# DefaultRui/VLN-VER

Measured on AMD Instinct MI355X. Metric: viewpoints/sec (multi-view->voxel fwd+bwd), vocc.py config, higher is better.
Workload: dtype bf16

## Files before the change

### include/ver_ops.h

```cpp
#ifndef VER_OPS_H
#define VER_OPS_H

#include <stdint.h>

#ifdef __cplusplus
extern "C" {
#endif

#define VER_ABI_VERSION 31

#define VER_OK            0
#define VER_EINVAL       -1
#define VER_EUNSUPPORTED -2
#define VER_ELAUNCH      -3

#define VER_F32  0
#define VER_BF16 1

int         ver_abi_version(void);
const char* ver_last_error(void);

int ver_msda_forward(const float* value, const int64_t* shapes_hw, const int64_t* level_start,
                     const float* loc, const float* attn_w, float* out,
                     int B, int num_keys, int heads, int head_dim, int levels, int points,
                     int Nq, int im2col_step, void* stream);

int ver_msda_backward(const float* value, const int64_t* shapes_hw, const int64_t* level_start,
                      const float* loc, const float* attn_w, const float* grad_out,
                      float* grad_value, float* grad_loc, float* grad_attn_w,
                      int B, int num_keys, int heads, int head_dim, int levels, int points,
                      int Nq, int im2col_step, void* stream);

int ver_msda3d_forward(const float* value, const int64_t* shapes_dhw, const int64_t* level_start,
                       const float* loc, const float* attn_w, float* out,
                       int B, int num_keys, int heads, int head_dim, int levels, int points,
                       int Nq, void* stream);
int ver_msda3d_backward(const float* value, const int64_t* shapes_dhw, const int64_t* level_start,
                        const float* loc, const float* attn_w, const float* grad_out,
                        float* grad_value, float* grad_loc, float* grad_attn_w,
                        int B, int num_keys, int heads, int head_dim, int levels, int points,
                        int Nq, void* stream);


int ver_project_points(const float* world2pixel, const float* origin, const float* pc_range,
                       int B, int Ncam, int bev_z, int bev_h, int bev_w,
                       float img_w, float img_h,
                       float* uv, uint8_t* vis, int32_t* vis_list, int32_t* vis_cnt,
                       int32_t* zero_list, int32_t* zero_cnt, int32_t* fwd_list, int32_t* fwd_cnt,
                       void* stream);

int ver_hits_from_mask(const uint8_t* bev_mask, int B, int Ncam, int Nq, int D,
                       uint8_t* vis, int32_t* vis_list, int32_t* vis_cnt,
                       int32_t* zero_list, int32_t* zero_cnt, int32_t* fwd_list, int32_t* fwd_cnt,
                       void* stream);

#define VER_SCA_ROWS_PREZEROED 1
#define VER_SCA_VALUE_HEAD_MAJOR 2
#define VER_SCA_GRAD_SLOTS_BF16 4
int ver_sca_head_major_supported(int value_dtype, int head_dim, int points, int map_h, int map_w);
int ver_sca_zero_rows(const int32_t* zero_list, const int32_t* zero_cnt, float* slots, int B, int Nq, int row_floats,
                      void* stream);
int ver_sca_forward(const void* value, int value_dtype, const float* offsets, const float* logits,
                    const float* uv, const uint8_t* vis, const int32_t* vis_list,
                    const int32_t* vis_cnt, const int32_t* zero_list, const int32_t* zero_cnt,
                    const int32_t* fwd_list, const int32_t* fwd_cnt,
                    float* slots,
                    int B, int Ncam, int Nq, int D, int heads, int head_dim, int points,
                    int map_h, int map_w, int flags, void* stream);

int ver_sca_backward_grad_dtype(int value_dtype, int head_dim, int points, int map_h, int map_w);
int ver_sca_backward(const void* value, int value_dtype, const float* offsets, const float* logits,
                     const float* uv, const uint8_t* vis, const int32_t* vis_list,
                     const int32_t* vis_cnt, const int32_t* fwd_list, const int32_t* fwd_cnt,
                     const void* grad_slots,
                     void* grad_value, int grad_value_dtype, float* grad_offsets, float* grad_logits,
                     int B, int Ncam, int Nq, int D, int heads, int head_dim, int points,
                     int map_h, int map_w, int flags, void* stream);

int ver_lattice_im2col(const void* src, void* col, const int* taps, int ntaps,
                       int B, int Z, int H, int W, int C, int dtype, void* stream);
int ver_lattice_col2im(const void* grad_col, void* grad_src, const int* taps, int ntaps,
                       int B, int Z, int H, int W, int C, int dtype, void* stream);

int ver_lattice_gather(const void* src, void* col, const int* taps, const long* col_offset, long col_stride,
                       int ntaps, int B, int Zr, int Zs, int H, int W, int C, int layout, int dtype,
                       const void* const_rows, const long* const_offset, int const_blocks, int const_width, void* stream);
int ver_lattice_scatter(const void* grad_col, void* grad_src, const int* taps, const long* col_offset,
                        long col_stride, int ntaps, int B, int Zr, int Zs, int H, int W, int C, int layout, int dtype,
                        void* stream);

int ver_convt_weight_forward(const float* weight, void* taps, long pairs, int dtype, void* stream);
int ver_convt_weight_backward(const void* grad_taps, float* grad_weight, long pairs, int dtype, void* stream);
int ver_convt_weight_backward_blocks(const void* blocks, const long* block_offsets, long ld, const void* prev_bias,
                                     const void* grad_v, float* grad_weight, int ci, int co, int dtype, void* stream);
int ver_convt_weight_forward_blocks(const float* weight, const long* block_offsets, long ld, void* blocks, int ci, int co,
                                    int dtype, void* stream);
int ver_blocks_vec_forward(const void* blocks, const long* block_rows, int nblocks, long ld, int ci, int ncols, const float* x,
                           float* vec, int dtype, void* stream);
int ver_blocks_vec_backward(const void* blocks, const long* block_rows, int nblocks, long ld, int ci, int ncols,
                            const float* grad_vec, float* grad_x, int dtype, void* stream);
int ver_lattice_transpose(void* channels_last, void* channel_first, long cf_stride, int B, int Z, int H, int W,
                          int C, int layout, int to_channel_first, int dtype, void* stream);
int ver_lattice_rows(void* channels_last, void* rows, long quarter, int period, int nseg, const int* seg_off,
                     const int* seg_len, const long* seg_base, const int* seg_pitch, const int* seg_rows, int B, int Z,
                     int H, int W, int C, int layout, int to_rows, int dtype, void* stream);

int ver_ln_relu_forward(const void* x, const float* gamma, const float* beta, void* y,
                        float* mean, float* rstd, long N, int W, float eps, int dtype, void* stream);
int ver_ln_relu_backward(const void* x, const void* grad_y, const float* gamma, const float* beta,
                         const float* mean, const float* rstd, void* grad_x,
                         float* grad_gamma, float* grad_beta, long N, int W, int dtype, void* stream);

int ver_focal_loss_blocks(long N, int C);
int ver_focal_loss_forward(const void* logits, const int64_t* target, float* partial, long N, int C,
                           float gamma, float alpha, int dtype, int32_t* bad_labels, void* stream);
int ver_focal_loss_forward_grad(const void* logits, const int64_t* target, float* partial, void* grad, long N, int C,
                                float gamma, float alpha, int dtype, int32_t* bad_labels, void* stream);
int ver_focal_loss_forward_grad_u8(const void* logits, const uint8_t* target, float* partial, void* grad, long N, int C,
                                   float gamma, float alpha, int dtype, int32_t* bad_labels, void* stream);
int ver_focal_loss_backward(const void* logits, const int64_t* target, const float* scale, void* grad,
                            long N, int C, float gamma, float alpha, int dtype, void* stream);

int ver_add_ln_forward(const void* a, int a_dtype, const float* residual, const float* gamma, const float* beta,
                       const int64_t* seed, float p_drop, float eps, float* y, void* y_bf16, float* mean,
                       float* rstd, long N, int C, void* stream);
int ver_add_ln_backward(const float* grad_y, const void* grad_y_bf16, const void* a, int a_dtype,
                        const float* residual, const float* gamma, const float* mean, const float* rstd,
                        const int64_t* seed, float p_drop, void* grad_a, float* grad_residual, float* grad_gamma,
                        float* grad_beta, long N, int C, void* stream);
int ver_relu_dropout_forward(const void* x, void* y, const int64_t* seed, float p_drop, long n, int dtype, void* stream);
int ver_relu_dropout_backward(const void* y, const void* grad_y, void* grad_x, float p_drop, long n, int dtype,
                              void* stream);

int ver_run_gather(const void* image, long image_stride, const int32_t* run_start, const int32_t* aug_idx,
                   void* rows, int B, int n_rows, int runs, int run_len, int n_aug, int row_elems, int dtype,
                   void* stream);
int ver_run_scatter(const void* rows, void* image, long image_stride, const int32_t* run_start, int B,
                    int n_rows, int runs, int run_len, int row_elems, int dtype, void* stream);

#define VER_OCC_MLP_CENTERED 2
long ver_occ_mlp_image_bytes(void);
int ver_occ_mlp_vector_floats(void);
int ver_occ_mlp_pack(const float* W1, const float* W2, const float* W3, void* image, void* stream);
int ver_occ_mlp_forward(const void* x, const void* image, const float* vectors, void* logits,
                        long N, int width, int classes, float eps, int first_linear, void* stream);
int ver_occ_mlp_forward_stats(const void* x, const void* image, const float* vectors, void* logits, float* rstd,
                              long N, int width, int classes, float eps, int first_linear, void* stream);
int ver_occ_mlp_backward(const void* x, const void* grad_logits, const void* image, const float* vectors,
                         void* grad_x, void* grad_a1, void* grad_a2, void* h1,
                         float* param_grads, long N, int width, int classes, float eps, int first_linear,
                         void* stream);
int ver_occ_mlp_backward_fused(const void* x, const void* grad_logits, const float* W2, const float* W3,
                               const float* vectors, void* grad_x, float* param_grads, long N, int width,
                               int classes, float eps, const float* grad_scale, int flags, void* stream);
int ver_occ_mlp_backward_fused_stats(const void* x, const void* grad_logits, const float* W2, const float* W3,
                                     const float* vectors, const float* rstd, void* grad_x, float* param_grads, long N,
                                     int width, int classes, float eps, const float* grad_scale, int flags, void* stream);

long ver_occ_predict_blocks(long N);
int  ver_occ_predict(const void* logits, int dtype, long N, int C, float threshold, int32_t* block_work,
                     int64_t* pairs, int64_t* count, void* stream);

int  ver_occ_confusion(const void* logits, int dtype, long rows_per_sample, int samples, int C, const uint8_t* labels,
                       const float* thresholds, int num_thresholds, int64_t* hist, void* stream);

int  ver_wgrad_tn_splits(long M, int Ka, int N);
int  ver_wgrad_tn_splits_ld(long M, int Ka, int N, long ld);
long ver_wgrad_tn_workspace(long M, int Ka, int N, int splits);
int  ver_wgrad_tn(const void* a, long lda, const void* g, long ldg, long M, int Ka, int N, void* out, long ldo,
                  int out_dtype, int splits, int flags, void* workspace, long workspace_bytes, void* stream);
int  ver_wgrad_tn_segments(const void* lattice, int layout, int B, int H, int W, int C, const int* taps, int nseg, const void* cst,
                           int ncst, int cw, const void* g, long ldg, int N, void* out, long ldo, int out_dtype, int splits,
                           void* workspace, long workspace_bytes, void* stream);
int  ver_wgrad_tn_segments_splits(int B, int H, int W, long Ka, int N, long ldg);

int  ver_gemm_nn(const void* a, long lda, const void* w, long ldw, const float* bias, void* c, long ldc, long M, int K,
                 int N, int flags, void* stream);
int  ver_gemm_nn_taps(const void* lattice, int layout, int B, int H, int W, int C, const int* taps, int ntaps, const void* w,
                      long ldw, const float* rowpos, const float* bias, void* c, long ldc, int N, void* stream);
int  ver_gemm_nn_segments(const void* lattice, int layout, int B, int H, int W, int C, const int* taps, int ntaps,
                          const void* cst, int ncst, int cw, const void* w, long ldw, const float* rowpos, const float* bias,
                          void* c, long ldc, int N, void* stream);
int  ver_gemm_nn_planes(const void* lattice, int layout, int B, int H, int W, int C, long plane_elems, int nplanes,
                        const int* tap_plane, const int* taps, int ntaps, const void* cst, int ncst, int cw, const void* w,
                        long ldw, const float* rowpos, const float* bias, void* c, long ldc, int N, void* stream);
int  ver_gemm_nn_splits(long M, int K, int N);
int  ver_gemm_nn_splitk(const void* a, long lda, const void* w, long ldw, const float* bias, void* c, long ldc, long M, int K,
                        int N, int splits, void* workspace, long workspace_bytes, void* stream);

int ver_clip_adamw_step(void* const* table, const long* sizes, const int* chunk_tensor, const int* chunk_index,
                        int n_tensors, int n_chunks, int chunk_elems, float* partial, float* norm_out, float max_norm,
                        float lr, float beta1, float beta2, float eps, float weight_decay, long step, void* stream);

int ver_clip_adamw_step_tensors(void* const* table, const long* sizes, const int* chunk_tensor, const int* chunk_index,
                                const float* hyper, int* steps, int n_tensors, int n_chunks, int chunk_elems, float* partial,
                                float* norm_out, float max_norm, void* stream);

int ver_lsa_solve(const float* cost, const int32_t* ncols, int32_t* match, int32_t* bad,
                  int P, int R, int Ccap, void* stream);

#ifdef __cplusplus
}
#endif
#endif
```

### vln-ver_amd/csrc/ver_wgrad.hip

```cpp
#include <cstdlib>
#include "ver_common.h"

namespace {
typedef __bf16 bf16x8 __attribute__((ext_vector_type(8)));
typedef float f32x16 __attribute__((ext_vector_type(16)));
typedef short s16x4 __attribute__((ext_vector_type(4)));
typedef short s16x8 __attribute__((ext_vector_type(8)));
typedef __attribute__((address_space(3))) s16x4 lds_s16x4;
typedef __attribute__((address_space(3))) void lds_void;

constexpr int kTile = 256;
constexpr int kSlabRows = 16;
constexpr int kSlabBytes = 2 * kSlabRows * kTile * 2;
constexpr int kRing = 8;
constexpr int kLdsBytes = kRing * kSlabBytes;

typedef int i32x2 __attribute__((ext_vector_type(2)));
typedef int i32x4 __attribute__((ext_vector_type(4)));

template <int OFF>
__device__ __forceinline__ i32x2 tr_read(int addr) {
    i32x2 v;
    asm volatile("ds_read_b64_tr_b16 %0, %1 offset:%2" : "=v"(v) : "v"(addr), "n"(OFF) : "memory");
    return v;
}
__device__ __forceinline__ bf16x8 frag(i32x2 lo, i32x2 hi) {
    return __builtin_bit_cast(bf16x8, (i32x4)__builtin_shufflevector(lo, hi, 0, 1, 2, 3));
}

struct WgradArgs {
    const __bf16* A;
    const __bf16* G;
    float* ws;
    long lda, ldg, M, Mc;
    int S, Ka, N, tiles_n, T;
    void* out;
    long ldo;
    int out_bf16;
    const __bf16* lattice;
    long lattice_bytes;
    const __bf16* cst;
    long cst_bytes;
    int B, H, W, C, P, CW, ncst, nseg;
    int seg_start[65];
    signed char kind[64], dz[64], dy[64], dx[64];
};

constexpr int kOutsideW = (int)0x80000000;
template <int L>
__device__ __forceinline__ int wcell_off(const WgradArgs& t, int b, int zl, int y, int x, int dz) {
    if ((unsigned)y >= (unsigned)t.H || (unsigned)x >= (unsigned)t.W) return kOutsideW;
    const int j = dz >> 1;
    int v;
    if (L == 0)
        v = ((b * 4 + zl + dz) * t.H + y) * t.W + x;
    else if (L == 2)
        v = ((((b * 2 + zl) * t.H + y) * t.W + x) << 1) + j;
    else
        v = (((((((y & 1) << 1 | (x & 1)) * t.B + b) * 2 + zl) * (t.H >> 1) + (y >> 1)) * (t.W >> 1) + (x >> 1)) << 1) + j;
    return v * t.C * 2;
}

struct WTapLane {
    int taddr;
    int boff;
    int bstep;
    int pend;
    int tend;
    int rows_left;
    int vo;
};

template <int L>
__device__ __forceinline__ int wtap_table_entry(const WgradArgs& t, int seg, int pos) {
    if (seg < 0) return kOutsideW;
    if (t.kind[seg]) return (pos * t.ncst + t.dz[seg]) * t.CW * 2;
    const int hw = t.H * t.W;
    const int zl = pos / hw, rem = pos - zl * hw;
    const int y = rem / t.W, x = rem - y * t.W;
    return wcell_off<L>(t, 0, zl, y + t.dy[seg], x + t.dx[seg], t.dz[seg]);
}

__device__ __forceinline__ int lds_read_b32(int addr) {
    int v;
    asm volatile("ds_read_b32 %0, %1" : "=v"(v) : "v"(addr) : "memory");
    return v;
}

__device__ __forceinline__ void wtap_step(const WgradArgs& t, WTapLane& tl, int tfetched) {
    tl.boff += tl.pend;
    tl.rows_left -= kSlabRows;
    tl.vo = tl.rows_left > 0 ? (int)((unsigned)tfetched + (unsigned)tl.boff) : kOutsideW;
    tl.taddr += 4 * kSlabRows;
    tl.pend = 0;
    if (tl.taddr >= tl.tend) tl.taddr -= 4 * t.P, tl.pend = tl.bstep;
}

struct WgradLane {
    int offA0, offA1, offB0, offB1;
    int voA, voG;
    int stepA, stepG;
    int dmaoff;
};

template <int SLOT>
__device__ __forceinline__ void read_slab(const WgradLane& c, i32x2 (&al)[4], i32x2 (&ah)[4], i32x2 (&bl)[2], i32x2 (&bh)[2]) {
    constexpr int SB = (SLOT & 3) * kSlabBytes;
    constexpr int UP = SLOT >= 4 ? 65536 : 0;
    const int a0 = c.offA0 + UP, a1 = c.offA1 + UP, b0 = c.offB0 + UP, b1 = c.offB1 + UP;
    al[0] = tr_read<SB>(a0);
    ah[0] = tr_read<SB + 512>(a0);
    bl[0] = tr_read<SB>(b0);
    bh[0] = tr_read<SB + 512>(b0);
    al[1] = tr_read<SB>(a1);
    ah[1] = tr_read<SB + 512>(a1);
    bl[1] = tr_read<SB>(b1);
    bh[1] = tr_read<SB + 512>(b1);
    al[2] = tr_read<SB + 1024>(a0);
    ah[2] = tr_read<SB + 1536>(a0);
    al[3] = tr_read<SB + 1024>(a1);
    ah[3] = tr_read<SB + 1536>(a1);
}

template <int PS, int KP, int PF, int IMPL>
__device__ __forceinline__ void phase(char* lds, f32x16 (&acc)[4][2], const WgradLane& c, __amdgpu_buffer_rsrc_t ra,
                                      __amdgpu_buffer_rsrc_t rg, unsigned& soA, unsigned& soG, const WgradArgs& t, WTapLane& tl) {
    i32x2 al[KP][4], ah[KP][4], bl[KP][2], bh[KP][2];
    int tnext = 0;
    read_slab<PS * KP>(c, al[0], ah[0], bl[0], bh[0]);
    if constexpr (KP == 2) read_slab<PS * KP + 1>(c, al[KP - 1], ah[KP - 1], bl[KP - 1], bh[KP - 1]);
#pragma unroll
    for (int u = 0; u < KP; ++u) {
        const int ds = (PS * KP + u + PF) % kRing;
        if constexpr (IMPL < 0) {
            __builtin_amdgcn_raw_ptr_buffer_load_lds(ra, (lds_void*)(lds + ds * kSlabBytes + c.dmaoff), 16, c.voA, (int)soA, 0, 0);
        } else {
            static_assert(IMPL < 0 || KP == 1, "implicit A: one slab per phase");
            __builtin_amdgcn_raw_ptr_buffer_load_lds(ra, (lds_void*)(lds + ds * kSlabBytes + c.dmaoff), 16, tl.vo, 0, 0, 0);
            tnext = lds_read_b32(tl.taddr);
        }
        __builtin_amdgcn_raw_ptr_buffer_load_lds(rg, (lds_void*)(lds + ds * kSlabBytes + kSlabBytes / 2 + c.dmaoff), 16, c.voG, (int)soG, 0, 0);
        soA += (unsigned)c.stepA;
        soG += (unsigned)c.stepG;
    }
    asm volatile("s_waitcnt vmcnt(%0)" ::"n"(2 * (PF - KP)) : "memory");
    __builtin_amdgcn_s_barrier();
    asm volatile("s_waitcnt lgkmcnt(0)"
                 : "+v"(al[0][0]), "+v"(ah[0][0]), "+v"(al[0][1]), "+v"(ah[0][1]), "+v"(al[0][2]), "+v"(ah[0][2]), "+v"(al[0][3]),
                   "+v"(ah[0][3]), "+v"(bl[0][0]), "+v"(bh[0][0]), "+v"(bl[0][1]), "+v"(bh[0][1]), "+v"(tnext)
                 :
                 : "memory");

    if constexpr (KP == 2)
        asm volatile(""
                     : "+v"(al[KP - 1][0]), "+v"(ah[KP - 1][0]), "+v"(al[KP - 1][1]), "+v"(ah[KP - 1][1]), "+v"(al[KP - 1][2]),
                       "+v"(ah[KP - 1][2]), "+v"(al[KP - 1][3]), "+v"(ah[KP - 1][3]), "+v"(bl[KP - 1][0]), "+v"(bh[KP - 1][0]),
                       "+v"(bl[KP - 1][1]), "+v"(bh[KP - 1][1])
                     :
                     : "memory");
    bf16x8 a[KP][4], b[KP][2];
#pragma unroll
    for (int u = 0; u < KP; ++u) {
#pragma unroll
        for (int i = 0; i < 4; ++i) a[u][i] = frag(al[u][i], ah[u][i]);
        b[u][0] = frag(bl[u][0], bh[u][0]);
        b[u][1] = frag(bl[u][1], bh[u][1]);
    }
    __builtin_amdgcn_sched_barrier(0);
    __builtin_amdgcn_s_setprio(1);
#pragma unroll
    for (int u = 0; u < KP; ++u)
#pragma unroll
        for (int it = 0; it < 4; ++it)
#pragma unroll
            for (int jt = 0; jt < 2; ++jt)
                acc[it][jt] = __builtin_amdgcn_mfma_f32_32x32x16_bf16(a[u][it], b[u][jt], acc[it][jt], 0, 0, 0);
    __builtin_amdgcn_s_setprio(0);
    __builtin_amdgcn_sched_barrier(0);
    if constexpr (IMPL >= 0) {
        wtap_step(t, tl, tnext);
        __builtin_amdgcn_sched_barrier(0);
    }
    __builtin_amdgcn_s_barrier();
}

template <int PS, int KP, int PF, int IMPL>
__device__ __forceinline__ void phases_from(int left, char* lds, f32x16 (&acc)[4][2], const WgradLane& c,
                                            __amdgpu_buffer_rsrc_t ra, __amdgpu_buffer_rsrc_t rg, unsigned& soA, unsigned& soG,
                                            const WgradArgs& t, WTapLane& tl) {
    if constexpr (PS < kRing / KP) {
        if (left > PS * KP) {
            phase<PS, KP, PF, IMPL>(lds, acc, c, ra, rg, soA, soG, t, tl);
            phases_from<PS + 1, KP, PF, IMPL>(left, lds, acc, c, ra, rg, soA, soG, t, tl);
        }
    }
}

template <int KP, int PF, int IMPL>
__device__ __forceinline__ void wgrad_body(const WgradArgs& p) {
    static_assert(PF >= KP && PF + (KP == 1 ? 2 : 4) <= kRing, "prefetch distance against the ring (WAR on the slot)");
    extern __shared__ __attribute__((aligned(1024))) char lds[];
    const int tid = threadIdx.x, lane = tid & 63;
    const int wave = __builtin_amdgcn_readfirstlane(tid >> 6);
    const int wr = wave >> 2, wc = wave & 3;
    int chunk, tile;
    {
        const int b = blockIdx.x;
        if ((p.S & 7) == 0) {
            const int xcd = b & 7, idx = b >> 3;
            chunk = xcd + 8 * (idx / p.T);
            tile = idx % p.T;
        } else {
            chunk = b / p.T;
            tile = b % p.T;
        }
    }
    const int mt = tile / p.tiles_n, nt = tile - mt * p.tiles_n;
    const long row0 = (long)chunk * p.Mc;
    const long rows = max(0L, min(p.Mc, p.M - row0));
    const int nslab = (int)((rows + kSlabRows * KP - 1) / (kSlabRows * KP)) * KP;

    const __bf16* ab = IMPL < 0 ? p.A + row0 * p.lda + (long)mt * kTile : nullptr;
    const __bf16* gb = p.G + row0 * p.ldg + (long)nt * kTile;
    const long abytes = ((p.M - row0 - 1) * p.lda + p.Ka - (long)mt * kTile) * 2;
    const long gbytes = ((p.M - row0 - 1) * p.ldg + p.N - (long)nt * kTile) * 2;
    const __amdgpu_buffer_rsrc_t rg = __builtin_amdgcn_make_buffer_rsrc((void*)gb, 0, (int)max(0L, min(gbytes, 0xFFFFFFFFL)), 0x00020000);
    WgradLane c;
    const int prow = lane >> 3, pch = (lane & 7) ^ (((prow >> 1) & 1) << 2);
    WTapLane tl = {};
    bool a_cst = false;
    if constexpr (IMPL >= 0) {
        int* tables = reinterpret_cast<int*>(lds + kLdsBytes);
        auto seg_of = [&](int col0) {
            int seg = -1;
            for (int i = 0; i < p.nseg; ++i)
                if (col0 >= p.seg_start[i] && col0 < p.seg_start[i + 1]) seg = i;
            return seg;
        };
        for (int q = 0; q < 4; ++q) {
            const int seg = seg_of(mt * kTile + 64 * q);
            for (int i = tid; i < p.P; i += 512) tables[q * p.P + i] = wtap_table_entry<IMPL>(p, seg, i);
        }
        __syncthreads();
        const int col0 = mt * kTile + 64 * (wave & 3);
        const int seg = seg_of(col0);
        a_cst = seg >= 0 && p.kind[seg];
        const long r = row0 + 8 * (wave >> 2) + prow;
        const int b0 = (int)(r / p.P), pos0 = (int)(r - (long)b0 * p.P);
        tl.bstep = a_cst ? 0 : (IMPL == 3 ? p.H * p.W : 4 * p.H * p.W) * p.C * 2;
        tl.boff = b0 * tl.bstep + (seg < 0 ? 0 : (col0 - p.seg_start[seg]) * 2) + pch * 16;
        const int lbase = (int)(uintptr_t)(__attribute__((address_space(3))) char*)(lds + kLdsBytes) + (wave & 3) * p.P * 4;
        tl.tend = lbase + 4 * p.P;
        tl.taddr = lbase + 4 * pos0;
        tl.pend = 0;
        tl.rows_left = (int)min(min(p.M, row0 + p.Mc) - r, 0x7FFFFFF0L) + kSlabRows;
        int t0 = lds_read_b32(tl.taddr);
        asm volatile("s_waitcnt lgkmcnt(0)" : "+v"(t0)::"memory");
        wtap_step(p, tl, t0);
    }
    const __amdgpu_buffer_rsrc_t ra =
        IMPL < 0 ? __builtin_amdgcn_make_buffer_rsrc((void*)ab, 0, (int)max(0L, min(abytes, 0xFFFFFFFFL)), 0x00020000)
                 : __builtin_amdgcn_make_buffer_rsrc((void*)(a_cst ? p.cst : p.lattice), 0,
                                                     (int)max(0L, min(a_cst ? p.cst_bytes : p.lattice_bytes, 0x7FFFFFFFL)), 0x00020000);
    c.voA = (int)(((8 * (wave >> 2) + prow) * p.lda + 64 * (wave & 3)) * 2) + pch * 16;
    c.voG = (int)(((8 * (wave >> 2) + prow) * p.ldg + 64 * (wave & 3)) * 2) + pch * 16;
    c.stepA = (int)(kSlabRows * p.lda * 2);
    c.stepG = (int)(kSlabRows * p.ldg * 2);
    c.dmaoff = wave * 1024;
    unsigned soA = 0, soG = 0;

    {
        const int q = lane >> 4, cl = lane & 15;
        const int lowch = (2 * (q & 1) + ((cl & 3) >> 1)) ^ (((cl >> 3) & 1) << 2);
        const int lbase = (int)(uintptr_t)(__attribute__((address_space(3))) char*)lds;
        const int rowoff = lbase + ((q >> 1) * 32 + (cl >> 2)) * 128 + lowch * 16 + (cl & 1) * 8;
        c.offA0 = rowoff + 2 * wr * 1024;
        c.offA1 = c.offA0 ^ 64;
        c.offB0 = rowoff + wc * 1024 + kSlabBytes / 2;
        c.offB1 = c.offB0 ^ 64;
    }

    f32x16 acc[4][2];
#pragma unroll
    for (int it = 0; it < 4; ++it)
#pragma unroll
        for (int jt = 0; jt < 2; ++jt)
#pragma unroll
            for (int r = 0; r < 16; ++r) acc[it][jt][r] = 0.0f;

#pragma unroll
    for (int s = 0; s < PF; ++s) {
        if constexpr (IMPL < 0) {
            __builtin_amdgcn_raw_ptr_buffer_load_lds(ra, (lds_void*)(lds + s * kSlabBytes + c.dmaoff), 16, c.voA, (int)soA, 0, 0);
        } else {
            __builtin_amdgcn_raw_ptr_buffer_load_lds(ra, (lds_void*)(lds + s * kSlabBytes + c.dmaoff), 16, tl.vo, 0, 0, 0);
            int tn = lds_read_b32(tl.taddr);
            asm volatile("s_waitcnt lgkmcnt(0)" : "+v"(tn)::"memory");
            wtap_step(p, tl, tn);
        }
        __builtin_amdgcn_raw_ptr_buffer_load_lds(rg, (lds_void*)(lds + s * kSlabBytes + kSlabBytes / 2 + c.dmaoff), 16, c.voG, (int)soG, 0, 0);
        soA += (unsigned)c.stepA;
        soG += (unsigned)c.stepG;
    }
    asm volatile("s_waitcnt vmcnt(%0)" ::"n"(2 * (PF - KP)) : "memory");
    __builtin_amdgcn_s_barrier();
    if (wr == 1) __builtin_amdgcn_s_barrier();

    int s = 0;
    for (; s + kRing <= nslab; s += kRing) phases_from<0, KP, PF, IMPL>(kRing, lds, acc, c, ra, rg, soA, soG, p, tl);
    phases_from<0, KP, PF, IMPL>(nslab - s, lds, acc, c, ra, rg, soA, soG, p, tl);
    if (wr == 0) __builtin_amdgcn_s_barrier();
    asm volatile("s_waitcnt vmcnt(0)" ::: "memory");

    const int i0 = mt * kTile + 128 * wr + 4 * (lane >> 5), j0 = nt * kTile + 64 * wc + (lane & 31);
    if (p.S == 1 && p.out) {
#pragma unroll
        for (int it = 0; it < 4; ++it)
#pragma unroll
            for (int jt = 0; jt < 2; ++jt) {
                const int j = j0 + 32 * jt;
#pragma unroll
                for (int r = 0; r < 16; ++r) {
                    const int i = i0 + 32 * it + (r & 3) + 8 * (r >> 2);
                    if (i < p.Ka && j < p.N) {
                        if (p.out_bf16)
                            reinterpret_cast<__bf16*>(p.out)[(long)i * p.ldo + j] = (__bf16)acc[it][jt][r];
                        else
                            reinterpret_cast<float*>(p.out)[(long)i * p.ldo + j] = acc[it][jt][r];
                    }
                }
            }
        return;
    }
    float* out = p.ws + (long)chunk * p.Ka * p.N;
#pragma unroll
    for (int it = 0; it < 4; ++it)
#pragma unroll
        for (int jt = 0; jt < 2; ++jt) {
            const int j = j0 + 32 * jt;
#pragma unroll
            for (int r = 0; r < 16; ++r) {
                const int i = i0 + 32 * it + (r & 3) + 8 * (r >> 2);
                if (i < p.Ka && j < p.N) out[(long)i * p.N + j] = acc[it][jt][r];
            }
        }
}

template <int KP, int PF>
__global__ __launch_bounds__(512) void k_wgrad_tn(WgradArgs p) {
    wgrad_body<KP, PF, -1>(p);
}

template <int L, int PF>
__global__ __launch_bounds__(512) void k_wgrad_tn_seg(WgradArgs p) {
    wgrad_body<1, PF, L>(p);
}

template <typename OT>
__global__ __launch_bounds__(256) void k_wgrad_reduce(const float* __restrict__ ws, OT* __restrict__ out, long ldo, int S,
                                                      int Ka, int N) {
    const long n4 = (long)Ka * N / 4;
    const long stride = (long)Ka * N;
    for (long e = blockIdx.x * 256L + threadIdx.x; e < n4; e += (long)gridDim.x * 256) {
        float4 acc = *reinterpret_cast<const float4*>(ws + 4 * e);
        for (int s = 1; s < S; ++s) {
            const float4 v = *reinterpret_cast<const float4*>(ws + s * stride + 4 * e);
            acc.x += v.x;
            acc.y += v.y;
            acc.z += v.z;
            acc.w += v.w;
        }
        const long i = (4 * e) / N, j = (4 * e) - i * N;
        OT* o = out + i * ldo + j;
        if constexpr (sizeof(OT) == 4) {
            *reinterpret_cast<float4*>(o) = acc;
        } else {
            typedef __bf16 bf16x4 __attribute__((ext_vector_type(4)));
            bf16x4 v;
            v.x = (__bf16)acc.x;
            v.y = (__bf16)acc.y;
            v.z = (__bf16)acc.z;
            v.w = (__bf16)acc.w;
            *reinterpret_cast<bf16x4*>(o) = v;
        }
    }
}

long max_chunk_rows(long ld) {
    if (ld <= 0) return 45000;
    const long rows = (0xFFFFFFFFL / (ld * 2)) - 16 * kRing - 2 * kSlabRows - 1;
    return rows < 45000 ? (rows > 2 * kSlabRows ? rows : 2 * kSlabRows) : 45000;
}

int pick_splits(long M, int Ka, int N, long ld = 0) {
    const long cap = max_chunk_rows(ld);
    const long tiles = (long)((Ka + kTile - 1) / kTile) * ((N + kTile - 1) / kTile);
    static const int cand[] = {1, 2, 3, 4, 6, 8, 12, 16, 24, 32, 48, 64};
    int best = 0;
    double best_us = 0.0;
    for (int s : cand) {
        if ((M + s - 1) / s > cap) continue;
        if (s > 1 && M / s < 256) break;
        if (M > 32768 && s % 8) continue;
        const long rounds = (tiles * s + 255) / 256;
        const double slabs = (double)((M + s - 1) / s + 15) / 16.0;
        double us = (double)rounds * (slabs * 0.37 + 8.0) + (s == 1 ? 0.25 : (double)s) * (double)Ka * (double)N * 8.0 / 3.0e6;
        if (s % 8 == 0) us *= 0.97;
        if (!best || us < best_us) {
            best = s;
            best_us = us;
        }
    }
    if (!best) {
        best = 64;
        while (best < 65536 && (M + best - 1) / best > cap) best *= 2;
    }
    return best;
}

template <int KP, int PF>
void launch_tn(const WgradArgs& p, int blocks, hipStream_t st, hipError_t& e) {
    auto kern = k_wgrad_tn<KP, PF>;
    e = hipFuncSetAttribute((const void*)kern, hipFuncAttributeMaxDynamicSharedMemorySize, kLdsBytes);
    if (e == hipSuccess) hipLaunchKernelGGL(kern, dim3((unsigned)blocks), dim3(512), kLdsBytes, st, p);
}
template <int L, int PF>
void launch_tn_segments_pf(const WgradArgs& p, int blocks, hipStream_t st, hipError_t& e) {
    const int ldsb = kLdsBytes + 4 * p.P * 4;
    e = hipFuncSetAttribute((const void*)k_wgrad_tn_seg<L, PF>, hipFuncAttributeMaxDynamicSharedMemorySize, ldsb);
    if (e == hipSuccess) hipLaunchKernelGGL((k_wgrad_tn_seg<L, PF>), dim3((unsigned)blocks), dim3(512), ldsb, st, p);
}

template <int L>
void launch_tn_segments(const WgradArgs& p, int blocks, hipStream_t st, hipError_t& e) {
    static const int pf = [] {
        const char* v = getenv("VER_WGRAD_SEG_PF");
        return v ? atoi(v) : 3;
    }();
    if (pf == 4) launch_tn_segments_pf<L, 4>(p, blocks, st, e);
    else if (pf == 5) launch_tn_segments_pf<L, 5>(p, blocks, st, e);
    else if (pf == 6) launch_tn_segments_pf<L, 6>(p, blocks, st, e);
    else launch_tn_segments_pf<L, 3>(p, blocks, st, e);
}
}

extern "C" int ver_wgrad_tn_splits(long M, int Ka, int N) {
    if (M <= 0 || Ka <= 0 || N <= 0) return 1;
    return pick_splits(M, Ka, N);
}

extern "C" int ver_wgrad_tn_splits_ld(long M, int Ka, int N, long ld) {
    if (M <= 0 || Ka <= 0 || N <= 0) return 1;
    return pick_splits(M, Ka, N, ld);
}

extern "C" long ver_wgrad_tn_workspace(long M, int Ka, int N, int splits) {
    if (Ka <= 0 || N <= 0) return 0;
    if (splits <= 0) splits = ver_wgrad_tn_splits(M, Ka, N);
    return (long)splits * Ka * N * (long)sizeof(float);
}

extern "C" int ver_wgrad_tn(const void* a, long lda, const void* g, long ldg, long M, int Ka, int N, void* out, long ldo,
                            int out_dtype, int splits, int flags, void* workspace, long workspace_bytes, void* stream) {
    hipStream_t st = (hipStream_t)stream;
    VER_REQUIRE(M >= 0 && Ka > 0 && N > 0, VER_EINVAL, "ver_wgrad_tn: bad sizes M=%ld Ka=%d N=%d", M, Ka, N);
    VER_REQUIRE(out && workspace && ((a && g) || M == 0), VER_EINVAL, "ver_wgrad_tn: null pointer argument");
    VER_REQUIRE(out_dtype == VER_F32 || out_dtype == VER_BF16, VER_EINVAL, "ver_wgrad_tn: out_dtype %d", out_dtype);
    VER_REQUIRE(lda >= Ka && ldg >= N && ldo >= N, VER_EINVAL, "ver_wgrad_tn: row pitch smaller than the row");
    VER_REQUIRE(lda % 8 == 0 && ldg % 8 == 0 && ((uintptr_t)a & 15) == 0 && ((uintptr_t)g & 15) == 0, VER_EUNSUPPORTED,
                "ver_wgrad_tn: operands must be 16-byte aligned with row pitches that are multiples of 8 elements");
    VER_REQUIRE(N % 4 == 0 && ldo % 4 == 0 && ((uintptr_t)out & 15) == 0, VER_EUNSUPPORTED,
                "ver_wgrad_tn: N and the output pitch must be multiples of 4");
    const int S = splits > 0 ? splits : pick_splits(M, Ka, N, lda > ldg ? lda : ldg);
    VER_REQUIRE(S <= 65536, VER_EINVAL, "ver_wgrad_tn: %d row chunks", S);
    const long Mc = ((M + S - 1) / S + 2 * kSlabRows - 1) / (2 * kSlabRows) * (2 * kSlabRows);
    VER_REQUIRE((Mc + 16 * kRing) * (lda > ldg ? lda : ldg) * 2 < 0xFFFFFFFFL, VER_EUNSUPPORTED,
                "ver_wgrad_tn: a row chunk exceeds the 4-GiB range of a buffer offset (more splits)");
    VER_REQUIRE(workspace_bytes >= (long)S * Ka * N * (long)sizeof(float), VER_EINVAL, "ver_wgrad_tn: workspace of %ld bytes, %ld needed",
                workspace_bytes, (long)S * Ka * N * (long)sizeof(float));
    WgradArgs p = {};
    p.A = (const __bf16*)a;
    p.G = (const __bf16*)g;
    p.ws = (float*)workspace;
    p.lda = lda;
    p.ldg = ldg;
    p.M = M;
    p.Mc = Mc;
    p.S = S;
    p.Ka = Ka;
    p.N = N;
    p.tiles_n = (N + kTile - 1) / kTile;
    p.T = ((Ka + kTile - 1) / kTile) * p.tiles_n;
    const bool direct = S == 1 && M > 0;
    p.out = direct ? out : nullptr;
    p.ldo = ldo;
    p.out_bf16 = out_dtype == VER_BF16;
    hipError_t e = hipSuccess;
    if (M > 0) {
        switch (flags & 15) {
            case 4: launch_tn<1, 4>(p, p.T * S, st, e); break;
            case 5: launch_tn<1, 5>(p, p.T * S, st, e); break;
            case 6: launch_tn<1, 6>(p, p.T * S, st, e); break;
            case 8 + 2: launch_tn<2, 2>(p, p.T * S, st, e); break;
            case 8 + 4: launch_tn<2, 4>(p, p.T * S, st, e); break;
            default: launch_tn<1, 3>(p, p.T * S, st, e); break;
        }
        if (e != hipSuccess) return ver_fail(VER_ELAUNCH, "ver_wgrad_tn: LDS attribute: %s", hipGetErrorString(e));
    } else if (int zrc = ver_zero_async(workspace, (size_t)S * Ka * N * sizeof(float), st)) {
        return zrc;
    }
    if (direct) return ver_check_launch("ver_wgrad_tn");
    const long n4 = (long)Ka * N / 4;
    long grid = (n4 + 255) / 256;
    if (grid > 8192) grid = 8192;
    if (out_dtype == VER_F32)
        hipLaunchKernelGGL(k_wgrad_reduce<float>, dim3((unsigned)grid), dim3(256), 0, st, (const float*)workspace, (float*)out, ldo, S, Ka, N);
    else
        hipLaunchKernelGGL(k_wgrad_reduce<__bf16>, dim3((unsigned)grid), dim3(256), 0, st, (const float*)workspace, (__bf16*)out, ldo, S, Ka, N);
    return ver_check_launch("ver_wgrad_tn");
}

extern "C" int ver_wgrad_tn_segments(const void* lattice, int layout, int B, int H, int W, int C, const int* taps, int nseg,
                                     const void* cst, int ncst, int cw, const void* g, long ldg, int N, void* out, long ldo,
                                     int out_dtype, int splits, void* workspace, long workspace_bytes, void* stream) {
    hipStream_t st = (hipStream_t)stream;
    VER_REQUIRE(B >= 0 && H > 0 && W > 0 && C > 0 && N > 0 && nseg > 0, VER_EINVAL, "ver_wgrad_tn_segments: bad sizes");
    VER_REQUIRE(layout == 0 || layout == 2 || layout == 3, VER_EINVAL, "ver_wgrad_tn_segments: layout %d (0 plain, 2 z-split, 3 planar z-split)", layout);
    VER_REQUIRE(layout != 3 || (H % 2 == 0 && W % 2 == 0), VER_EINVAL, "ver_wgrad_tn_segments: planar needs even H, W");
    VER_REQUIRE(out && workspace && ((lattice && g && taps) || B == 0), VER_EINVAL, "ver_wgrad_tn_segments: null pointer argument");
    VER_REQUIRE(out_dtype == VER_F32 || out_dtype == VER_BF16, VER_EINVAL, "ver_wgrad_tn_segments: out_dtype %d", out_dtype);
    VER_REQUIRE(nseg <= 64, VER_EUNSUPPORTED, "ver_wgrad_tn_segments: %d segments (at most 64)", nseg);
    VER_REQUIRE(C % 64 == 0 && (cst == nullptr || (ncst > 0 && ncst <= 64 && cw > 0 && cw % 64 == 0 && ((uintptr_t)cst & 15) == 0)),
                VER_EUNSUPPORTED, "ver_wgrad_tn_segments: segment widths (C = %d, pattern blocks of %d) must be multiples of 64", C, cw);
    const long M = (long)B * 2 * H * W, lbytes = (long)B * 4 * H * W * C * 2;
    const int P = 2 * H * W;
    VER_REQUIRE(P >= kSlabRows && P <= 2048 && lbytes < 0x7FFFFFFFL, VER_EUNSUPPORTED,
                "ver_wgrad_tn_segments: %d rows per viewpoint / a source lattice of %ld bytes (16 <= rows <= 2048: four offset tables "
                "next to the 128-KB ring in LDS; below 2 GiB)", P, lbytes);
    VER_REQUIRE(ldg >= N && ldo >= N && ldg % 8 == 0 && ((uintptr_t)g & 15) == 0 && ((uintptr_t)lattice & 15) == 0, VER_EUNSUPPORTED,
                "ver_wgrad_tn_segments: g must be 16-byte aligned with a row pitch that is a multiple of 8 elements");
    VER_REQUIRE(N % 4 == 0 && ldo % 4 == 0 && ((uintptr_t)out & 15) == 0, VER_EUNSUPPORTED,
                "ver_wgrad_tn_segments: N and the output pitch must be multiples of 4");
    WgradArgs p = {};
    long Ka = 0;
    for (int i = 0; i < nseg; ++i) {
        const int dz = taps[3 * i], dy = taps[3 * i + 1], dx = taps[3 * i + 2];
        p.seg_start[i] = (int)Ka;
        if (dz < 0) {
            VER_REQUIRE(cst && -1 - dz < ncst, VER_EINVAL, "ver_wgrad_tn_segments: segment %d names pattern block %d of %d", i, -1 - dz, cst ? ncst : 0);
            p.kind[i] = 1, p.dz[i] = (signed char)(-1 - dz);
            Ka += cw;
        } else {
            VER_REQUIRE((dz == 0 || dz == 2) && dy >= -64 && dy <= 64 && dx >= -64 && dx <= 64, VER_EINVAL,
                        "ver_wgrad_tn_segments: tap %d = (%d, %d, %d): dz must be 0 or 2", i, dz, dy, dx);
            p.kind[i] = 0, p.dz[i] = (signed char)dz, p.dy[i] = (signed char)dy, p.dx[i] = (signed char)dx;
            Ka += C;
        }
    }
    p.seg_start[nseg] = (int)Ka;
    VER_REQUIRE(Ka < 0x7FFFFFFFL, VER_EUNSUPPORTED, "ver_wgrad_tn_segments: %ld columns", Ka);
    const int S = splits > 0 ? splits : pick_splits(M, (int)Ka, N, ldg);
    VER_REQUIRE(S <= 65536, VER_EINVAL, "ver_wgrad_tn_segments: %d row chunks", S);
    const long Mc = ((M + S - 1) / S + 2 * kSlabRows - 1) / (2 * kSlabRows) * (2 * kSlabRows);
    VER_REQUIRE((Mc + 16 * kRing) * ldg * 2 < 0xFFFFFFFFL, VER_EUNSUPPORTED,
                "ver_wgrad_tn_segments: a row chunk exceeds the 4-GiB range of a buffer offset (more splits)");
    VER_REQUIRE(workspace_bytes >= (long)S * Ka * N * (long)sizeof(float), VER_EINVAL, "ver_wgrad_tn_segments: workspace of %ld bytes, %ld needed",
                workspace_bytes, (long)S * Ka * N * (long)sizeof(float));
    p.A = nullptr;
    p.G = (const __bf16*)g;
    p.ws = (float*)workspace;
    p.lda = 0;
    p.ldg = ldg;
    p.M = M;
    p.Mc = Mc;
    p.S = S;
    p.Ka = (int)Ka;
    p.N = N;
    p.tiles_n = (N + kTile - 1) / kTile;
    p.T = (int)((Ka + kTile - 1) / kTile) * p.tiles_n;
    const bool direct = S == 1 && M > 0;
    p.out = direct ? out : nullptr;
    p.ldo = ldo;
    p.out_bf16 = out_dtype == VER_BF16;
    p.lattice = (const __bf16*)lattice;
    p.lattice_bytes = lbytes;
    p.cst = (const __bf16*)cst;
    p.cst_bytes = cst ? (long)P * ncst * cw * 2 : 0;
    p.B = B, p.H = H, p.W = W, p.C = C, p.P = P, p.CW = cw, p.ncst = ncst, p.nseg = nseg;
    hipError_t e = hipSuccess;
    if (M > 0) {
        if (layout == 0) launch_tn_segments<0>(p, p.T * S, st, e);
        else if (layout == 2) launch_tn_segments<2>(p, p.T * S, st, e);
        else launch_tn_segments<3>(p, p.T * S, st, e);
        if (e != hipSuccess) return ver_fail(VER_ELAUNCH, "ver_wgrad_tn_segments: LDS attribute: %s", hipGetErrorString(e));
    } else if (int zrc = ver_zero_async(workspace, (size_t)S * Ka * N * sizeof(float), st)) {
        return zrc;
    }
    if (direct) return ver_check_launch("ver_wgrad_tn_segments");
    const long n4 = Ka * N / 4;
    long grid = (n4 + 255) / 256;
    if (grid > 8192) grid = 8192;
    if (out_dtype == VER_F32)
        hipLaunchKernelGGL(k_wgrad_reduce<float>, dim3((unsigned)grid), dim3(256), 0, st, (const float*)workspace, (float*)out, ldo, S, (int)Ka, N);
    else
        hipLaunchKernelGGL(k_wgrad_reduce<__bf16>, dim3((unsigned)grid), dim3(256), 0, st, (const float*)workspace, (__bf16*)out, ldo, S, (int)Ka, N);
    return ver_check_launch("ver_wgrad_tn_segments");
}

extern "C" int ver_wgrad_tn_segments_splits(int B, int H, int W, long Ka, int N, long ldg) {
    const long M = (long)B * 2 * H * W;
    if (M <= 0 || Ka <= 0 || N <= 0) return 1;
    return pick_splits(M, (int)Ka, N, ldg);
}
```

### vln-ver_amd/dense_heads/upsample.py

```python
import os

import torch

from . import _cpu_algebra
from ._cpu_algebra import ZS_PLAIN, ZS_PLANAR_SPLIT, ZS_SPLIT, planar_to_plain, planar_zs_to_plain, zs_to_plain
from ._cpu_algebra import plain_to_planar
from .lattice_plan import (_CLASSES, _COLS3, _COLS4, _PW, _PW2, _aug_rows_z4, _block_offsets, _class_patterns, _class_rows_z4,
                           _class_segments_z4, _const_rows_z4, _dgrad_plan, _layer0_z4_plan, _layer_plan, _layer_plan_z4,
                           _stack_tables_z4)

KERNEL = (3, 5, 5)
GEOM = dict(stride=(1, 2, 2), padding=(2, 4, 4), dilation=(2, 2, 2), output_padding=(0, 1, 1))
_HIP_DTYPES = (torch.float32, torch.bfloat16)


class _HipAlgebra:

    @staticmethod
    def corr_weight(weight, dtype):
        if weight.dtype == torch.float32 and dtype in _HIP_DTYPES:
            from ..hipops import convt_weight_taps
            return convt_weight_taps(weight, dtype)
        return _cpu_algebra.corr_weight(weight, dtype)

    @staticmethod
    def im2col(e, taps):
        from ..hipops import lattice_im2col
        return lattice_im2col(e.contiguous(), taps)

    @staticmethod
    def gather27(e, planar, a_mat, ci, hc, wc, taps, offs):
        from ..hipops import lattice_gather
        lattice_gather(e.contiguous(), a_mat, taps, offs, (hc, wc), 1 if planar else 0)

    @staticmethod
    def scatter27(d_a, planar, shape, ci, hc, wc, taps, offs):
        from ..hipops import lattice_scatter
        return lattice_scatter(d_a, d_a.new_empty(shape), taps, offs, (hc, wc), 1 if planar else 0)

    @staticmethod
    def gather_z4(e, layout, a_mat, taps, offs, ci, hc, wc, const=None):
        from ..hipops import lattice_gather
        if const is not None and e.dtype in _HIP_DTYPES:
            lattice_gather(e.contiguous(), a_mat, taps, offs, (hc, wc), layout, row_z=2, const_rows=const[0], const_offset=const[1])
            return True
        lattice_gather(e.contiguous(), a_mat, taps, offs, (hc, wc), layout, row_z=2)
        return False

    @staticmethod
    def scatter_z4(d_a, layout, shape, taps, offs, ci, hc, wc):
        from ..hipops import lattice_scatter
        return lattice_scatter(d_a, d_a.new_empty(shape), taps, offs, (hc, wc), layout, row_z=2)

    @staticmethod
    def channels_last(x0, dt):
        b, c, z, h, w = x0.shape
        pos = z * h * w
        if dt in _HIP_DTYPES:
            vx = 4 if dt == torch.bfloat16 else 2
            for wd in range(min(pos, 120), 0, -1):
                if pos % wd == 0 and wd % vx == 0:
                    return _ChannelsLast.apply(x0, dt, (pos // wd, wd))
        return _cpu_algebra.channels_last(x0, dt)


def _algebra(t):
    return _HipAlgebra if t.is_cuda else _cpu_algebra


def _on_hip(t):
    return _algebra(t) is _HipAlgebra


def is_reference_geometry(conv):
    return (tuple(conv.kernel_size) == KERNEL and tuple(conv.stride) == GEOM['stride'] and
            tuple(conv.padding) == GEOM['padding'] and tuple(conv.dilation) == GEOM['dilation'] and
            tuple(conv.output_padding) == GEOM['output_padding'] and conv.groups == 1)


_to_plain, _from_plain = _cpu_algebra.to_plain, _cpu_algebra.from_plain


def _corr_weight(weight, dtype):
    return _algebra(weight).corr_weight(weight, dtype)


def _im2col(e, taps):
    return _algebra(e).im2col(e, taps)


def _bias_through_taps(prev_bias, k):
    t, ci, _ = k.shape
    return torch.bmm(prev_bias.view(1, 1, ci).expand(t, 1, ci).contiguous(), k).squeeze(1)


def _stacked_rows(k, bias, prev_bias, total_rows):
    _, ci, co = k.shape
    v = _bias_through_taps(prev_bias.to(k.dtype), k)
    vaug = torch.cat([v, bias.to(k.dtype)[None], v.new_zeros(_PW - 76, co)])
    return torch.cat([k.reshape(75 * ci, co), vaug, vaug, vaug, vaug, v.new_zeros(total_rows - 75 * ci - 4 * _PW, co)])


def _stacked_rows_backward(d_rows, k, prev_bias):
    _, ci, co = k.shape
    dt = k.dtype
    n_data = 75 * ci
    acc = torch.float64 if dt == torch.float64 else torch.float32
    d_vaug = d_rows[n_data:n_data + 4 * _PW].view(4, _PW, co).sum(0, dtype=acc)
    d_v = d_vaug[:75].to(dt)
    d_k = torch.addcmul(d_rows[:n_data].view(75, ci, co), prev_bias.to(dt)[None, :, None], d_v[:, None, :])
    d_prev = torch.bmm(k, d_v.unsqueeze(2)).sum(0).squeeze(1)
    return d_k, d_vaug[75].to(prev_bias.dtype), d_prev.to(prev_bias.dtype)


def _layer0(e, k, bias):
    b, z, h, w, c = e.shape
    taps = [(2 * a - 2, bb - 2, cc - 2) for a in range(3) for bb in range(5) for cc in range(5)]
    a_mat = _im2col(e, taps)
    out = torch.addmm(bias, a_mat, k.reshape(75 * c, -1))
    return out.view(b, z, h, w, -1)


def _gather27(e, planar, a_mat, ci, hc, wc):
    _algebra(e).gather27(e, planar, a_mat, ci, hc, wc, _COLS3.taps, _COLS3.block_offsets(ci))


def _scatter27(d_a, planar, shape, ci, hc, wc):
    return _algebra(d_a).scatter27(d_a, planar, shape, ci, hc, wc, _COLS3.taps, _COLS3.block_offsets(ci))


class _LatticeLayer(torch.autograd.Function):

    @staticmethod
    def forward(ctx, e, k, bias, prev_bias, planar):
        if planar:
            _, b, z, hh, wh, ci = e.shape
            hc, wc = 2 * hh, 2 * wh
        else:
            b, z, hc, wc, ci = e.shape
        co = k.shape[-1]
        plan, kt, total_rows = _layer_plan(ci, e.device)
        m = b * z * hc * wc
        a_mat = e.new_empty(m, kt)
        _gather27(e, planar, a_mat, ci, hc, wc)
        a3 = a_mat.view(b, z * hc * wc, kt)
        for cls, pat in zip(_CLASSES, _class_patterns(z, hc, wc, e.device, e.dtype)):
            o = _COLS3.const_offset(cls, ci)
            a3[:, :, o:o + _PW] = pat
        rows = _stacked_rows(k, bias, prev_bias, total_rows)
        out = e.new_empty(4, m, co)
        for p, cls in enumerate(_CLASSES):
            c0, c1, ridx = plan[cls]
            torch.mm(a_mat[:, c0:c1], rows.index_select(0, ridx), out=out[p])
        ctx.save_for_backward(a_mat, rows, k, prev_bias)
        ctx.geom = (planar, tuple(e.shape), hc, wc)
        return out.view(4, b, z, hc, wc, co)

    @staticmethod
    def backward(ctx, grad_out):
        a_mat, rows, k, prev_bias = ctx.saved_tensors
        planar, e_shape, hc, wc = ctx.geom
        _, ci, co = k.shape
        plan, kt, total_rows = _layer_plan(ci, a_mat.device)
        m = a_mat.shape[0]
        g = grad_out.contiguous().view(4, m, co)
        d_a = a_mat.new_empty(m, kt)
        d_a[:, kt - _PW:] = 0
        d_rows = rows.new_empty(total_rows, co)
        for p, cls in enumerate(_CLASSES):
            c0, c1, ridx = plan[cls]
            w = rows.index_select(0, ridx)
            if p == 0:
                torch.mm(g[p], w.t(), out=d_a[:, c0:c1])
            else:
                torch.addmm(d_a[:, c0:c1], g[p], w.t(), out=d_a[:, c0:c1])
            d_rows.index_copy_(0, ridx, rows_tn(a_mat[:, c0:c1], g[p]))
        d_e = _scatter27(d_a, planar, e_shape, ci, hc, wc)
        return (d_e, *_stacked_rows_backward(d_rows, k, prev_bias), None)


def _gather_z4(e, layout, a_mat, taps, offs, ci, hc, wc, with_const=False):
    const = _const_rows_z4(ci, hc, wc, e.device, e.dtype) if with_const else None
    return _algebra(e).gather_z4(e, layout, a_mat, taps, offs, ci, hc, wc, const)


def _scatter_z4(d_a, layout, shape, taps, offs, ci, hc, wc):
    return _algebra(d_a).scatter_z4(d_a, layout, shape, taps, offs, ci, hc, wc)


_IMPLICIT_TAPS = os.environ.get('VER_IMPLICIT_TAPS', '1') != '0'


def _implicit_taps(e, layout, rows, combined_hw, ci, raw, const_width):
    if not (_IMPLICIT_TAPS and _OWN_GEMM and raw is not None and _on_hip(e) and e.dtype == torch.bfloat16 and rows >= _OWN_GEMM_MIN_ROWS):
        return False
    from ..hipops import gemm_nn_taps_supported, wgrad_tn_segments_supported
    return gemm_nn_taps_supported(e, layout, None, ci) and wgrad_tn_segments_supported(e, layout, combined_hw, ci, const_width, None)


def _dgrad_implicit(kind, g_planes, weights, b, hc, wc, ci, co):
    from ..hipops import gemm_nn_taps
    lat = g_planes.view(g_planes.shape[0], b, 2, hc, wc, 2, co)
    rows, taps, planes, nb = _dgrad_plan(kind, ci, g_planes.device)
    wcat = weights.index_select(0, rows).view(nb, 2 * ci, 2 * co).transpose(1, 2).reshape(nb * 2 * co, 2 * ci)
    d_e = gemm_nn_taps(lat if kind != 'l0' else lat[0], ZS_SPLIT, (hc, wc), taps, wcat, planes=planes if kind != 'l0' else None,
                       timer_class='head_gemm_dgrad')
    return d_e.view(b, 2, hc, wc, 2, ci)


def _dgrad_explicit_l0(g, wmat, shape, taps, offs, ci, h, w):
    with gemm_timed('head_gemm_dgrad', g.shape[0], g.shape[1], wmat.shape[0]):
        d_a = torch.mm(g, wmat.t())
    return _scatter_z4(d_a, ZS_PLAIN, shape, taps, offs, ci, h, w)


class _Layer0Z4Taps(torch.autograd.Function):

    @staticmethod
    def forward(ctx, x, k, bias):
        b, _, h, w, ci = x.shape
        co = k.shape[-1]
        taps, offs, lo, hi = _layer0_z4_plan(ci, x.device)
        a_mat = x.new_empty(b * 2 * h * w, 50 * ci)
        _gather_z4(x, ZS_PLAIN, a_mat, taps, offs, ci, h, w)
        rows = k.reshape(75 * ci, co)
        wmat = torch.cat([rows.index_select(0, lo), rows.index_select(0, hi)], 1)
        out = mm_fwd(a_mat, wmat, bias=torch.cat([bias, bias]))
        ctx.save_for_backward(a_mat, wmat)
        ctx.geom = (tuple(x.shape), ci, co, h, w)
        return out.view(b, 2, h, w, 2, co)

    @staticmethod
    def backward(ctx, grad_out):
        a_mat, wmat = ctx.saved_tensors
        shape, ci, co, h, w = ctx.geom
        taps, offs, lo, hi = _layer0_z4_plan(ci, a_mat.device)
        g = grad_out.contiguous().view(-1, 2 * co)
        d_x = _dgrad_explicit_l0(g, wmat, shape, taps, offs, ci, h, w)
        d_w = rows_tn(a_mat, g)
        d_b = g.sum(0, dtype=torch.float64 if g.dtype == torch.float64 else torch.float32)
        d_lo = d_w.new_zeros(75 * ci, co)
        d_hi = d_w.new_zeros(75 * ci, co)
        d_lo.index_copy_(0, lo, d_w[:, :co])
        d_hi.index_copy_(0, hi, d_w[:, co:])
        return d_x, (d_lo + d_hi).view(75, ci, co), (d_b[:co] + d_b[co:]).to(g.dtype)


class _Layer0Z4Raw(torch.autograd.Function):

    @staticmethod
    def forward(ctx, x, raw, bias):
        from ..hipops import convt_weight_forward_blocks
        b, _, h, w, ci = x.shape
        co = raw.shape[1]
        taps, offs, _, _ = _layer0_z4_plan(ci, x.device)
        ctx.implicit = _implicit_taps(x, ZS_PLAIN, b * 2 * h * w, (h, w), ci, raw, 0)
        if ctx.implicit:
            operand = x.contiguous()
        else:
            operand = x.new_empty(b * 2 * h * w, 50 * ci)
            _gather_z4(x, ZS_PLAIN, operand, taps, offs, ci, h, w)
        wmat = convt_weight_forward_blocks(raw, _block_offsets('l0', ci, co, x.device), x.new_empty(50 * ci, 2 * co), ci, co)
        bias2 = torch.cat([bias, bias])
        if ctx.implicit:
            from ..hipops import gemm_nn_taps
            out = gemm_nn_taps(operand, ZS_PLAIN, (h, w), taps, wmat, bias=bias2.to(x.dtype).float())
        else:
            out = mm_fwd(operand, wmat, bias=bias2)
        ctx.save_for_backward(operand, wmat)
        ctx.geom = (tuple(x.shape), ci, co, h, w)
        return out.view(b, 2, h, w, 2, co)

    @staticmethod
    def backward(ctx, grad_out):
        from ..hipops import convt_weight_backward_blocks
        operand, wmat = ctx.saved_tensors
        shape, ci, co, h, w = ctx.geom
        taps, offs, _, _ = _layer0_z4_plan(ci, operand.device)
        g = grad_out.contiguous().view(-1, 2 * co)
        if ctx.implicit:
            from ..hipops import wgrad_tn_segments
            d_x = zs_to_plain(_dgrad_implicit('l0', g[None], wmat, shape[0], h, w, ci, co))
            d_w = wgrad_tn_segments(operand, ZS_PLAIN, (h, w), taps, g)
        else:
            d_x = _dgrad_explicit_l0(g, wmat, shape, taps, offs, ci, h, w)
            d_w = rows_tn(operand, g)
        d_b = g.sum(0, dtype=torch.float32)
        d_raw = convt_weight_backward_blocks(d_w, _block_offsets('l0', ci, co, d_w.device), None, None, ci, co)
        return d_x, d_raw, (d_b[:co] + d_b[co:]).to(g.dtype)


def _geom_z4(e, planar):
    if planar:
        _, b, _, hh, wh, _, ci = e.shape
        return ZS_PLANAR_SPLIT, b, 2 * hh, 2 * wh, ci
    b, _, hc, wc, _, ci = e.shape
    return ZS_SPLIT, b, hc, wc, ci


def _tap_matrix_z4(e, layout, b, hc, wc, ci):
    _, kt, _, taps, offs = _layer_plan_z4(ci, e.device)
    a_mat = e.new_empty(b * 2 * hc * wc, kt)
    if not _gather_z4(e, layout, a_mat, taps, offs, ci, hc, wc, with_const=True):
        a3 = a_mat.view(b, 2 * hc * wc, kt)
        for cls, pat in zip(_CLASSES, _class_patterns(4, hc, wc, e.device, e.dtype)):
            o = _COLS4.const_offset(cls, ci)
            halves = pat.view(2, 2 * hc * wc, _PW)
            a3[:, :, o:o + _PW] = halves[0]
            a3[:, :, o + _PW:o + _PW2] = halves[1]
    return a_mat


def _class_ranges_z4(ci, device):
    plan, rows = _layer_plan_z4(ci, device)[0], _class_rows_z4(ci)
    ranges = [(plan[cls][0], plan[cls][1], rows[cls][0], rows[cls][0] + plan[cls][1] - plan[cls][0]) for cls in _CLASSES]
    return ranges, ranges[-1][3]


def _dgrad_class(d_a, p, g_p, w, c0, c1):
    with gemm_timed('head_gemm_dgrad', g_p.shape[0], g_p.shape[1], c1 - c0):
        if p == 0:
            torch.mm(g_p, w.t(), out=d_a[:, c0:c1])
        else:
            torch.addmm(d_a[:, c0:c1], g_p, w.t(), out=d_a[:, c0:c1])


class _LatticeLayerZ4Taps(torch.autograd.Function):

    @staticmethod
    def forward(ctx, e, k, bias, prev_bias, planar):
        layout, b, hc, wc, ci = _geom_z4(e, planar)
        co = k.shape[-1]
        plan, _, total_rows, _, _ = _layer_plan_z4(ci, e.device)
        a_mat = _tap_matrix_z4(e, layout, b, hc, wc, ci)
        out = e.new_empty(4, a_mat.shape[0], 2 * co)
        rows = _stacked_rows(k, bias, prev_bias, total_rows)
        ws = []
        for p, cls in enumerate(_CLASSES):
            c0, c1, _, _, lohi = plan[cls]
            ws.append(rows.index_select(0, lohi).view(c1 - c0, 2 * co))
            mm_fwd(a_mat[:, c0:c1], ws[p], out=out[p])
        ctx.save_for_backward(a_mat, k, prev_bias, *ws)
        ctx.geom = (layout, tuple(e.shape), hc, wc)
        return out.view(4, b, 2, hc, wc, 2, co)

    @staticmethod
    def backward(ctx, grad_out):
        a_mat, k, prev_bias, *ws = ctx.saved_tensors
        layout, e_shape, hc, wc = ctx.geom
        _, ci, co = k.shape
        plan, kt, total_rows, taps, offs = _layer_plan_z4(ci, a_mat.device)
        m = a_mat.shape[0]
        g = grad_out.contiguous().view(4, m, 2 * co)
        d_a = a_mat.new_empty(m, kt)
        d_a[:, kt - _PW2:] = 0
        d_lo = a_mat.new_zeros(total_rows, co)
        d_hi = a_mat.new_zeros(total_rows, co)
        for p, cls in enumerate(_CLASSES):
            c0, c1, lo, hi, _ = plan[cls]
            _dgrad_class(d_a, p, g[p], ws[p], c0, c1)
            d_w = rows_tn(a_mat[:, c0:c1], g[p])
            d_lo.index_copy_(0, lo, d_w[:, :co])
            d_hi.index_copy_(0, hi, d_w[:, co:])
        d_e = _scatter_z4(d_a, layout, e_shape, taps, offs, ci, hc, wc)
        del d_a
        return (d_e, *_stacked_rows_backward(d_lo + d_hi, k, prev_bias), None)


class _LatticeLayerZ4Raw(torch.autograd.Function):

    @staticmethod
    def forward(ctx, e, raw, bias, prev_bias, planar):
        from ..hipops import blocks_vec_forward, convt_weight_forward_blocks
        layout, b, hc, wc, ci = _geom_z4(e, planar)
        co = raw.shape[1]
        dt = e.dtype
        m = b * 2 * hc * wc
        ctx.implicit = _implicit_taps(e, layout, m, (hc, wc), ci, raw, _PW2)
        operand = e.contiguous() if ctx.implicit else _tap_matrix_z4(e, layout, b, hc, wc, ci)
        out = e.new_empty(4, m, 2 * co)
        ranges, n_rows = _class_ranges_z4(ci, e.device)
        block_rows, tap_slot, const_rows, const_src = _stack_tables_z4(ci, e.device)
        stack = e.new_empty(n_rows, 2 * co)
        convt_weight_forward_blocks(raw, _block_offsets('lat', ci, co, e.device), stack, ci, co)
        v = blocks_vec_forward(stack, block_rows, ci, prev_bias).view(-1, co).index_select(0, tap_slot)
        vaug = torch.cat([v.to(dt), bias.to(dt)[None], v.new_zeros(_PW - 75, co, dtype=dt)])
        stack.view(-1, co).index_copy_(0, const_rows, vaug.index_select(0, const_src))
        for p, (cls, (c0, c1, r0, r1)) in enumerate(zip(_CLASSES, ranges)):
            if ctx.implicit:
                from ..hipops import gemm_nn_taps
                gemm_nn_taps(operand, layout, (hc, wc), _class_segments_z4(cls, ci), stack[r0:r1],
                             const_rows=_const_rows_z4(ci, hc, wc, e.device, dt)[0], out=out[p])
            else:
                mm_fwd(operand[:, c0:c1], stack[r0:r1], out=out[p])
        ctx.save_for_backward(operand, stack, prev_bias)
        ctx.geom = (layout, tuple(e.shape), b, hc, wc, ci, co)
        return out.view(4, b, 2, hc, wc, 2, co)

    @staticmethod
    def backward(ctx, grad_out):
        from ..hipops import blocks_vec_backward, convt_weight_backward_blocks
        operand, stack, prev_bias = ctx.saved_tensors
        layout, e_shape, b, hc, wc, ci, co = ctx.geom
        _, kt, _, taps, offs = _layer_plan_z4(ci, operand.device)
        ranges, n_rows = _class_ranges_z4(ci, operand.device)
        dt = operand.dtype
        m = b * 2 * hc * wc
        g = grad_out.contiguous().view(4, m, 2 * co)
        if not ctx.implicit:
            d_a = operand.new_empty(m, kt)
            d_a[:, kt - _PW2:] = 0
        d_stack = operand.new_empty(n_rows, 2 * co)
        for p, (cls, (c0, c1, r0, r1)) in enumerate(zip(_CLASSES, ranges)):
            if ctx.implicit:
                from ..hipops import wgrad_tn_segments
                wgrad_tn_segments(operand, layout, (hc, wc), _class_segments_z4(cls, ci), g[p], out=d_stack[r0:r1],
                                  const_rows=_const_rows_z4(ci, hc, wc, operand.device, dt)[0])
            else:
                _dgrad_class(d_a, p, g[p], stack[r0:r1], c0, c1)
                rows_tn(operand[:, c0:c1], g[p], out=d_stack[r0:r1])
        if ctx.implicit:
            d_e = _dgrad_implicit('lat', g, stack, b, hc, wc, ci, co)
            if layout == ZS_PLANAR_SPLIT:
                d_e = d_e.view(b, 2, hc // 2, 2, wc // 2, 2, 2, ci).permute(3, 5, 0, 1, 2, 4, 6, 7).reshape(e_shape)
        else:
            d_e = _scatter_z4(d_a, layout, e_shape, taps, offs, ci, hc, wc)
            del d_a
        own = d_stack.view(-1, co).index_select(0, _aug_rows_z4(ci, d_stack.device)).view(8, _PW, co)
        d_vaug = own.sum(0, dtype=torch.float32)
        d_v = d_vaug[:75].to(dt)
        pb = prev_bias.to(dt)
        d_raw = convt_weight_backward_blocks(d_stack, _block_offsets('lat', ci, co, d_stack.device), pb, d_v, ci, co)
        block_rows, tap_slot, _, _ = _stack_tables_z4(ci, d_stack.device)
        dv2 = d_vaug.new_zeros(2 * block_rows.numel(), co).index_copy_(0, tap_slot, d_vaug[:75])
        d_prev = blocks_vec_backward(stack, block_rows, ci, dv2.view(block_rows.numel(), 2 * co))
        return d_e, d_raw, d_vaug[75].to(prev_bias.dtype), d_prev.to(prev_bias.dtype), None


class _Layer0Z4:

    @staticmethod
    def apply(x, k, bias, raw=None):
        return _Layer0Z4Taps.apply(x, k, bias) if raw is None else _Layer0Z4Raw.apply(x, raw, bias)


class _LatticeLayerZ4:

    @staticmethod
    def apply(e, k, bias, prev_bias, planar, raw=None):
        if raw is None:
            return _LatticeLayerZ4Taps.apply(e, k, bias, prev_bias, planar)
        return _LatticeLayerZ4Raw.apply(e, raw, bias, prev_bias, planar)


def gemm_timed(name, m, k, n):
    from ..hipops import timed
    return timed(name, 2.0 * m * k * n)


_OWN_GEMM = os.environ.get('VER_OWN_GEMM', '1') == '1'
_OWN_GEMM_MIN_ROWS = int(os.environ.get('VER_OWN_GEMM_MIN_ROWS', '14000'))
_OWN_GEMM_SKINNY_ROWS = 2048


def mm_fwd(a, w, out=None, bias=None):
    m, k = a.shape
    n = w.shape[1]
    if _OWN_GEMM and _on_hip(a) and a.dtype == torch.bfloat16 and w.dtype == torch.bfloat16 and k >= 2048 and \
            (m >= _OWN_GEMM_MIN_ROWS or m <= _OWN_GEMM_SKINNY_ROWS):
        from ..hipops import gemm_nn, gemm_nn_splits, gemm_nn_supported
        if gemm_nn_supported(a, w) and (out is None or (out.stride(-1) == 1 and out.dtype == torch.bfloat16)) and \
                (m >= _OWN_GEMM_MIN_ROWS or gemm_nn_splits(m, k, n) > 1):
            return gemm_nn(a, w, None if bias is None else bias.to(a.dtype).float(), out)
    with gemm_timed('head_gemm_fwd', m, k, n):
        if bias is None:
            return torch.mm(a, w, out=out) if out is not None else torch.mm(a, w)
        b = bias.to(a.dtype)
        return torch.addmm(b, a, w, out=out) if out is not None else torch.addmm(b, a, w)


def rows_tn(a, g, out_dtype=None, out=None):
    if _on_hip(a) and a.dtype == torch.bfloat16 and g.dtype == torch.bfloat16:
        from ..hipops import wgrad_tn, wgrad_tn_supported
        if g.stride(-1) != 1 or g.stride(0) % 8:
            g = g.contiguous()
        if wgrad_tn_supported(a, g):
            return wgrad_tn(a, g, out_dtype=out_dtype if out is None else out.dtype, out=out)
    if out is not None:
        return torch.mm(a.t(), g, out=out) if out.dtype == a.dtype else out.copy_(torch.mm(a.t(), g))
    res = torch.mm(a.t(), g)
    return res if out_dtype is None else res.to(out_dtype)


def _compute_dtype(x):
    if _on_hip(x) and torch.is_autocast_enabled('cuda'):
        return torch.get_autocast_dtype('cuda')
    return x.dtype


class _ChannelsLast(torch.autograd.Function):

    @staticmethod
    def forward(ctx, x0, dt, split):
        from ..hipops import lattice_transpose
        b, c, z, h, w = x0.shape
        cf = x0.to(dt).contiguous().view(b, c * z * h * w)
        e = torch.empty(b, z, h, w, c, dtype=dt, device=x0.device)
        lattice_transpose(e.view(b, 1, split[0], split[1], c), cf, split, 0, False)
        ctx.split, ctx.in_dtype = split, x0.dtype
        return e

    @staticmethod
    def backward(ctx, g):
        from ..hipops import lattice_transpose
        b, z, h, w, c = g.shape
        g = g.contiguous()
        cf = torch.empty(b, c * z * h * w, dtype=g.dtype, device=g.device)
        lattice_transpose(g.view(b, 1, ctx.split[0], ctx.split[1], c), cf, ctx.split, 0, True)
        return cf.view(b, c, z, h, w).to(ctx.in_dtype), None, None


def _channels_last(x0, dt):
    return _algebra(x0).channels_last(x0, dt)


def upsample_lattice(x0, weights, biases):
    dt = _compute_dtype(x0)
    e = _channels_last(x0, dt)
    bs = [b.to(dt) for b in biases]
    if e.shape[1] == 4 and _on_hip(e) and dt in _HIP_DTYPES and all(_on_hip(w) and w.dtype == torch.float32 for w in weights):
        e = _Layer0Z4.apply(e, None, bs[0], weights[0])
        e = _LatticeLayerZ4.apply(e, None, bs[1], bs[0], False, weights[1])
        e = _LatticeLayerZ4.apply(e, None, bs[2], bs[1], True, weights[2])
        return e, bs[2]
    ks = [_corr_weight(w, dt) for w in weights]
    if e.shape[1] == 4:
        e = _Layer0Z4.apply(e, ks[0], bs[0])
        e = _LatticeLayerZ4.apply(e, ks[1], bs[1], bs[0], False)
        e = _LatticeLayerZ4.apply(e, ks[2], bs[2], bs[1], True)
        return e, bs[2]
    e = _layer0(e, ks[0], bs[0])
    e = _LatticeLayer.apply(e, ks[1], bs[1], bs[0], False)
    e = _LatticeLayer.apply(e, ks[2], bs[2], bs[1], True)
    return e, bs[2]


def full_volume(e, bias):
    if e.dim() == 7:
        e = planar_zs_to_plain(e)
    elif e.dim() == 6:
        e = planar_to_plain(e)
    b, z, h, w, c = e.shape
    y = bias.view(1, c, 1, 1, 1).expand(b, c, z, 2 * h, 2 * w).contiguous()
    y[:, :, :, ::2, ::2] = e.permute(0, 4, 1, 2, 3)
    return y


def upsample_dense(x0, weights, biases):
    e, b = upsample_lattice(x0, weights, biases)
    return full_volume(e, b)
```

### vln-ver_amd/hipops.py

```python
import ctypes
import os
import re

import torch
from torch.autograd import Function
from torch.autograd.function import once_differentiable

_PKG = os.path.dirname(os.path.abspath(__file__))
LIB_PATH = os.environ.get('VER_HIP_LIB') or os.path.join(_PKG, 'libver_hip.so')
ABI_VERSION = 31
HEADER = os.path.join(os.path.dirname(_PKG), 'include', 'ver_ops.h')
_PARAMS = {'int': ctypes.c_int, 'long': ctypes.c_long, 'float': ctypes.c_float}
_RETURNS = {'int': ctypes.c_int, 'long': ctypes.c_long, 'const char*': ctypes.c_char_p}


class HipLibraryError(RuntimeError):
    pass


def prototypes(path=HEADER):
    if not os.path.exists(path):
        raise HipLibraryError('%s not found: the C ABI is bound from its prototypes' % path)
    text = re.sub(r'/\*.*?\*/|//[^\n]*|^\s*#[^\n]*', ' ', open(path).read(), flags=re.S | re.M)
    out = {}
    for ret, name, params in re.findall(r'([^;{}()]*?)\b(ver_[a-z0-9_]+)\s*\(([^()]*)\)\s*;', text):
        ret = _RETURNS.get(' '.join(ret.split()))
        params = [] if params.strip() == 'void' else [' '.join(q.split()) for q in params.split(',')]
        args = [ctypes.c_void_p if '*' in q else _PARAMS.get(q.rpartition(' ')[0]) for q in params]
        if ret is None or None in args:
            raise HipLibraryError('%s: %s(%s): a type outside int / long / float / pointer' % (path, name, ', '.join(params)))
        out[name] = (ret, args)
    unread = set(re.findall(r'\b(ver_[a-z0-9_]+)\s*\(', text)) - set(out)
    if unread:
        raise HipLibraryError('%s: no prototype read for %s' % (path, ', '.join(sorted(unread))))
    return out


PROTOTYPES = prototypes()
SYMBOLS = tuple(PROTOTYPES)

_lib = None


def lib():
    global _lib
    if _lib is None:
        if not os.path.exists(LIB_PATH):
            raise HipLibraryError(
                '%s not found: build it with `python -c "import __graft_entry__ as g; g.build()"` '
                '(hipcc --offload-arch=gfx950). There is no CPU/PyTorch fallback.' % LIB_PATH)
        handle = ctypes.CDLL(LIB_PATH)
        for name, (ret, params) in PROTOTYPES.items():
            if not hasattr(handle, name):
                raise HipLibraryError('%s does not export %s' % (LIB_PATH, name))
            fn = getattr(handle, name)
            fn.restype, fn.argtypes = ret, params
        if handle.ver_abi_version() != ABI_VERSION:
            raise HipLibraryError('libver_hip.so ABI %d != expected %d: rebuild'
                                  % (handle.ver_abi_version(), ABI_VERSION))
        _lib = handle
    return _lib


def _check(rc, what):
    if rc != 0:
        msg = lib().ver_last_error()
        raise RuntimeError('%s failed (%d): %s' % (what, rc, msg.decode() if msg else ''))


class KernelTimer:

    def __init__(self):
        self.records = []

    def summary(self):
        torch.cuda.synchronize()
        out = {}
        for name, e0, e1, meta in self.records:
            d = out.setdefault(name, dict(count=0, ms=0.0, flops=0.0, meta=meta))
            d['count'] += 1
            d['ms'] += e0.elapsed_time(e1)
            if meta and 'flops' in meta:
                d['flops'] += meta['flops']
        return out


KERNEL_TIMER = None


def _launch(name, fn, meta=None):
    timer = KERNEL_TIMER
    if timer is None:
        return _check(fn(), name)
    e0 = torch.cuda.Event(enable_timing=True)
    e1 = torch.cuda.Event(enable_timing=True)
    e0.record()
    rc = fn()
    e1.record()
    timer.records.append((name, e0, e1, meta))
    return _check(rc, name)


class timed:

    def __init__(self, name, flops=0.0):
        self.name, self.flops = name, flops

    def __enter__(self):
        self.timer = KERNEL_TIMER
        if self.timer is not None:
            self.e0 = torch.cuda.Event(enable_timing=True)
            self.e0.record()
        return self

    def __exit__(self, *exc):
        if self.timer is not None:
            e1 = torch.cuda.Event(enable_timing=True)
            e1.record()
            self.timer.records.append((self.name, self.e0, e1, dict(flops=self.flops)))
        return False


def _p(t):
    return None if t is None else t.data_ptr()


def _stream():
    return torch.cuda.current_stream().cuda_stream


def _gpu(t, name, dtype=None):
    if not t.is_cuda:
        raise RuntimeError('%s must be a GPU tensor: the VER ops only exist as HIP kernels' % name)
    if dtype is not None and t.dtype != dtype:
        raise TypeError('%s must be %s, got %s' % (name, dtype, t.dtype))
    return t.contiguous()


class MultiScaleDeformableAttnFunction_fp32(Function):

    @staticmethod
    @torch.amp.custom_fwd(device_type='cuda', cast_inputs=torch.float32)
    def forward(ctx, value, value_spatial_shapes, value_level_start_index, sampling_locations,
                attention_weights, im2col_step):
        value = _gpu(value, 'value', torch.float32)
        loc = _gpu(sampling_locations, 'sampling_locations', torch.float32)
        aw = _gpu(attention_weights, 'attention_weights', torch.float32)
        shapes = _gpu(value_spatial_shapes, 'value_spatial_shapes').to(torch.int64)
        lsi = _gpu(value_level_start_index, 'value_level_start_index').to(torch.int64)
        bs, nk, heads, hd = value.shape
        _, nq, _, nl, npt, _ = loc.shape
        ctx.im2col_step = im2col_step
        out = value.new_empty(bs, nq, heads * hd)
        _check(lib().ver_msda_forward(_p(value), _p(shapes), _p(lsi), _p(loc), _p(aw), _p(out),
                                      bs, nk, heads, hd, nl, npt, nq, im2col_step, _stream()),
               'ver_msda_forward')
        ctx.save_for_backward(value, shapes, lsi, loc, aw)
        return out

    @staticmethod
    @once_differentiable
    @torch.amp.custom_bwd(device_type='cuda')
    def backward(ctx, grad_output):
        value, shapes, lsi, loc, aw = ctx.saved_tensors
        bs, nk, heads, hd = value.shape
        _, nq, _, nl, npt, _ = loc.shape
        grad_value = torch.zeros_like(value)
        grad_loc = torch.zeros_like(loc)
        grad_aw = torch.zeros_like(aw)
        go = _gpu(grad_output, 'grad_output').float().contiguous()
        _check(lib().ver_msda_backward(_p(value), _p(shapes), _p(lsi), _p(loc), _p(aw), _p(go),
                                       _p(grad_value), _p(grad_loc), _p(grad_aw), bs, nk, heads, hd,
                                       nl, npt, nq, ctx.im2col_step, _stream()),
               'ver_msda_backward')
        return grad_value, None, None, grad_loc, grad_aw, None


MultiScaleDeformableAttnFunction_fp16 = MultiScaleDeformableAttnFunction_fp32


class HitTable:

    __slots__ = ('uv', 'vis', 'vis_list', 'vis_cnt', 'zero_list', 'zero_cnt', 'fwd_list', 'fwd_cnt',
                 'B', 'Ncam', 'Nq', 'D')

    def __init__(self, B, Ncam, Nq, D, device):
        self.B, self.Ncam, self.Nq, self.D = B, Ncam, Nq, D
        self.uv = torch.empty(B, Ncam, Nq, D, 2, dtype=torch.float32, device=device)
        self.vis = torch.empty(B, Nq, dtype=torch.uint8, device=device)
        self.vis_list = torch.empty(B, Ncam, Nq, dtype=torch.int32, device=device)
        self.vis_cnt = torch.empty(B, Ncam, dtype=torch.int32, device=device)
        self.zero_list = torch.empty(B, Nq, dtype=torch.int32, device=device)
        self.zero_cnt = torch.empty(B, dtype=torch.int32, device=device)
        self.fwd_list = torch.empty(B, Ncam, Nq, dtype=torch.int32, device=device)
        self.fwd_cnt = torch.empty(B, Ncam, 2, dtype=torch.int32, device=device)

    def mask(self):
        bits = torch.arange(self.Ncam, device=self.vis.device, dtype=torch.uint8)
        m = (self.vis[None] >> bits[:, None, None]) & 1
        return m.bool().unsqueeze(-1)


def project_points(world2pixel, origin, pc_range, bev_z, bev_h, bev_w, img_w=1280.0, img_h=1024.0):
    w2p = _gpu(world2pixel, 'world2pixel', torch.float32)
    org = _gpu(origin, 'origin', torch.float32)
    B, ncam = w2p.shape[0], w2p.shape[1]
    nq = bev_z * bev_h * bev_w
    hit = HitTable(B, ncam, nq, 1, w2p.device)
    rng = (ctypes.c_float * 6)(*[float(v) for v in pc_range])
    _launch('ver_project_points', lambda: lib().ver_project_points(
        _p(w2p), _p(org), rng, B, ncam, bev_z, bev_h, bev_w, img_w, img_h,
        _p(hit.uv), _p(hit.vis), _p(hit.vis_list), _p(hit.vis_cnt), _p(hit.zero_list), _p(hit.zero_cnt),
        _p(hit.fwd_list), _p(hit.fwd_cnt), _stream()))
    return hit


def hits_from_mask(reference_points_cam, bev_mask):
    ncam, B, nq, D = bev_mask.shape
    mask = _gpu(bev_mask, 'bev_mask').to(torch.uint8).contiguous()
    hit = HitTable(B, ncam, nq, D, mask.device)
    hit.uv.copy_(reference_points_cam.to(torch.float32).permute(1, 0, 2, 3, 4))
    _check(lib().ver_hits_from_mask(_p(mask), B, ncam, nq, D, _p(hit.vis), _p(hit.vis_list),
                                    _p(hit.vis_cnt), _p(hit.zero_list), _p(hit.zero_cnt), _p(hit.fwd_list),
                                    _p(hit.fwd_cnt), _stream()),
           'ver_hits_from_mask')
    return hit


_SIDE_STREAMS = {}
SCA_PREZERO = os.environ.get('VER_SCA_PREZERO', '1') != '0'


def _side_stream(device):
    st = _SIDE_STREAMS.get(device)
    if st is None:
        st = _SIDE_STREAMS[device] = torch.cuda.Stream(device=device)
    return st


class PreparedSlots:
    __slots__ = ('slots', 'done')

    def __init__(self, slots, done):
        self.slots, self.done = slots, done


def sca_prepare_slots(hit, row_floats):
    if not SCA_PREZERO or torch.cuda.is_current_stream_capturing():
        return None
    dev = hit.vis.device
    slots = torch.empty(hit.B, hit.Nq, row_floats, dtype=torch.float32, device=dev)
    main, side = torch.cuda.current_stream(dev), _side_stream(dev)
    side.wait_stream(main)
    slots.record_stream(side)
    with torch.cuda.stream(side):
        _launch('ver_sca_zero_rows', lambda: lib().ver_sca_zero_rows(
            _p(hit.zero_list), _p(hit.zero_cnt), _p(slots), hit.B, hit.Nq, row_floats, _stream()))
        done = torch.cuda.Event()
        done.record(side)
    return PreparedSlots(slots, done)


class SCAGatherFunction(Function):

    @staticmethod
    def forward(ctx, value, offsets, logits, hit, map_h, map_w, prepared=None, head_major=False, lowp_out=False):
        if value.dtype not in (torch.float32, torch.bfloat16):
            value = value.float()
        value = _gpu(value, 'value')
        offsets = _gpu(offsets, 'offsets').float().contiguous()
        logits = _gpu(logits, 'logits').float().contiguous()
        vdt = 1 if value.dtype == torch.bfloat16 else 0
        if head_major:
            heads, B, ncam, nk, hd = value.shape
        else:
            B, ncam, nk, heads, hd = value.shape
        points = logits.shape[-1]
        nq = hit.Nq
        assert nk == map_h * map_w and B == hit.B and ncam == hit.Ncam
        assert offsets.shape == (B, nq, heads, points, 2) and logits.shape == (B, nq, heads, points)
        flags = 2 if head_major else 0
        if prepared is not None:
            slots = prepared.slots
            assert slots.shape == (B, nq, heads * hd) and slots.dtype == torch.float32 and slots.is_contiguous()
            with timed('ver_sca_zero_wait'):
                torch.cuda.current_stream(slots.device).wait_event(prepared.done)
            with timed('ver_event_floor'):
                pass
            flags |= 1
        else:
            slots = torch.empty(B, nq, heads * hd, dtype=torch.float32, device=value.device)
        _launch('ver_sca_forward', lambda: lib().ver_sca_forward(
            _p(value), vdt, _p(offsets), _p(logits), _p(hit.uv), _p(hit.vis), _p(hit.vis_list),
            _p(hit.vis_cnt), _p(hit.zero_list), _p(hit.zero_cnt), _p(hit.fwd_list), _p(hit.fwd_cnt), _p(slots),
            B, ncam, nq, hit.D, heads, hd,
            points, map_h, map_w, flags, _stream()), meta=dict(prezeroed=bool(flags & 1), head_major=head_major))
        ctx.save_for_backward(value, offsets, logits)
        ctx.hit, ctx.map_hw, ctx.vdt, ctx.head_major = hit, (map_h, map_w), vdt, head_major
        if lowp_out and vdt == 1:
            return slots.to(torch.bfloat16)
        return slots

    @staticmethod
    @once_differentiable
    def backward(ctx, grad_slots):
        value, offsets, logits = ctx.saved_tensors
        hit = ctx.hit
        map_h, map_w = ctx.map_hw
        if ctx.head_major:
            heads, B, ncam, nk, hd = value.shape
        else:
            B, ncam, nk, heads, hd = value.shape
        points = logits.shape[-1]
        gdt = lib().ver_sca_backward_grad_dtype(ctx.vdt, hd, points, map_h, map_w)
        gs = _gpu(grad_slots, 'grad_slots')
        gs_bf16 = gs.dtype == torch.bfloat16 and gdt == 1
        gs = gs.contiguous() if gs_bf16 else gs.float().contiguous()
        g_value = torch.empty((B, ncam, nk, heads, hd), dtype=torch.bfloat16 if gdt == 1 else torch.float32, device=value.device)
        g_off = torch.empty_like(offsets)
        g_log = torch.empty_like(logits)
        _launch('ver_sca_backward', lambda: lib().ver_sca_backward(
            _p(value), ctx.vdt, _p(offsets), _p(logits), _p(hit.uv), _p(hit.vis), _p(hit.vis_list),
            _p(hit.vis_cnt), _p(hit.fwd_list), _p(hit.fwd_cnt), _p(gs), _p(g_value), gdt, _p(g_off), _p(g_log), B, ncam,
            hit.Nq, hit.D, heads,
            hd, points, map_h, map_w, (2 if ctx.head_major else 0) | (4 if gs_bf16 else 0), _stream()),
            meta=dict(grad_slots_bf16=gs_bf16))
        g_value = g_value.to(value.dtype)
        if ctx.head_major:
            g_value = g_value.permute(3, 0, 1, 2, 4)
        return g_value, g_off, g_log, None, None, None, None, None, None


def sca_gather(value, offsets, logits, hit, map_h, map_w, prepared=None, head_major=False, lowp_out=False):
    return SCAGatherFunction.apply(value, offsets, logits, hit, map_h, map_w, prepared, head_major, lowp_out)


def sca_head_major_supported(dtype, head_dim, points, map_h, map_w):
    return dtype == torch.bfloat16 and bool(lib().ver_sca_head_major_supported(1, head_dim, points, map_h, map_w))


class HeadMajorLinearFunction(Function):

    @staticmethod
    def forward(ctx, x, weight, bias, heads):
        m, c_in = x.shape
        w = weight.to(x.dtype)
        hd = w.shape[0] // heads
        out = x.new_empty(heads, m, hd)
        b = bias.to(x.dtype).view(heads, hd)
        w3 = w.view(heads, hd, c_in)
        for h in range(heads):
            torch.addmm(b[h], x, w3[h].t(), out=out[h])
        ctx.save_for_backward(x, w)
        ctx.heads = heads
        return out

    @staticmethod
    @once_differentiable
    def backward(ctx, g):
        x, w = ctx.saved_tensors
        heads = ctx.heads
        m = x.shape[0]
        g2 = g.permute(1, 0, 2).reshape(m, -1)
        from .dense_heads.upsample import rows_tn
        dw = rows_tn(g2, x) if ctx.needs_input_grad[1] else None
        db = g2.sum(0, dtype=torch.float32) if ctx.needs_input_grad[2] else None
        dx = g2 @ w if ctx.needs_input_grad[0] else None
        return dx, dw, db, None


def head_major_linear(x, weight, bias, heads):
    return HeadMajorLinearFunction.apply(x, weight, bias, heads)


class LatticeIm2colFunction(Function):

    @staticmethod
    def forward(ctx, lattice, taps):
        lattice = _gpu(lattice, 'lattice')
        if lattice.dtype not in (torch.float32, torch.bfloat16):
            raise TypeError('lattice must be fp32 or bf16')
        B, Z, H, W, C = lattice.shape
        flat = [int(v) for t in taps for v in t]
        arr = (ctypes.c_int * len(flat))(*flat)
        dt = 1 if lattice.dtype == torch.bfloat16 else 0
        col = torch.empty(B * Z * H * W, len(taps) * C, dtype=lattice.dtype, device=lattice.device)
        _launch('ver_lattice_im2col', lambda: lib().ver_lattice_im2col(
            _p(lattice), _p(col), arr, len(taps), B, Z, H, W, C, dt, _stream()))
        ctx.geom = (B, Z, H, W, C, dt, arr, len(taps))
        return col

    @staticmethod
    @once_differentiable
    def backward(ctx, grad_col):
        B, Z, H, W, C, dt, arr, ntaps = ctx.geom
        want = torch.bfloat16 if dt else torch.float32
        g = _gpu(grad_col, 'grad_col').to(want).contiguous()
        grad = torch.empty(B, Z, H, W, C, dtype=want, device=g.device)
        _launch('ver_lattice_col2im', lambda: lib().ver_lattice_col2im(
            _p(g), _p(grad), arr, ntaps, B, Z, H, W, C, dt, _stream()))
        return grad, None


def lattice_im2col(lattice, taps):
    return LatticeIm2colFunction.apply(lattice, taps)


class ConvTWeightFunction(Function):

    @staticmethod
    def forward(ctx, weight, dtype):
        weight = _gpu(weight, 'weight')
        if weight.dtype != torch.float32 or tuple(weight.shape[2:]) != (3, 5, 5):
            raise TypeError('weight must be fp32 [Ci,Co,3,5,5]')
        if dtype not in (torch.float32, torch.bfloat16):
            raise TypeError('taps dtype must be fp32 or bf16')
        weight = weight.contiguous()
        ci, co = weight.shape[:2]
        taps = torch.empty(75, ci, co, dtype=dtype, device=weight.device)
        dt = 1 if dtype == torch.bfloat16 else 0
        _launch('ver_convt_weight_forward', lambda: lib().ver_convt_weight_forward(
            _p(weight), _p(taps), ci * co, dt, _stream()))
        ctx.shape, ctx.dt, ctx.dtype = tuple(weight.shape), dt, dtype
        return taps

    @staticmethod
    @once_differentiable
    def backward(ctx, grad_taps):
        g = _gpu(grad_taps, 'grad_taps').to(ctx.dtype).contiguous()
        ci, co = ctx.shape[:2]
        gw = torch.empty(ctx.shape, dtype=torch.float32, device=g.device)
        _launch('ver_convt_weight_backward', lambda: lib().ver_convt_weight_backward(
            _p(g), _p(gw), ci * co, ctx.dt, _stream()))
        return gw, None


def convt_weight_taps(weight, dtype):
    return ConvTWeightFunction.apply(weight, dtype)


def convt_weight_backward_blocks(blocks, block_offsets, prev_bias, grad_v, ci, co):
    src = _gpu(blocks, 'blocks')
    if src.dim() != 2 or src.stride(1) != 1 or src.dtype not in (torch.float32, torch.bfloat16):
        raise TypeError('convt_weight_backward_blocks: blocks must be an fp32 / bf16 matrix with unit column stride')
    off = _gpu(block_offsets, 'block_offsets')
    if off.dtype != torch.int64 or tuple(off.shape) != (75, 2) or not off.is_contiguous():
        raise TypeError('convt_weight_backward_blocks: block_offsets must be a contiguous int64 [75, 2]')
    if (prev_bias is None) != (grad_v is None):
        raise ValueError('convt_weight_backward_blocks: prev_bias and grad_v come together')
    if prev_bias is not None:
        prev_bias = _gpu(prev_bias, 'prev_bias').to(src.dtype).contiguous()
        grad_v = _gpu(grad_v, 'grad_v').to(src.dtype).contiguous()
        if prev_bias.numel() != ci or tuple(grad_v.shape) != (75, co):
            raise ValueError('convt_weight_backward_blocks: prev_bias [Ci] and grad_v [75, Co] expected')
    gw = torch.empty(ci, co, 3, 5, 5, dtype=torch.float32, device=src.device)
    dt = 1 if src.dtype == torch.bfloat16 else 0
    _launch('ver_convt_weight_backward_blocks', lambda: lib().ver_convt_weight_backward_blocks(
        _p(src), _p(off), src.stride(0), _p(prev_bias), _p(grad_v), _p(gw), ci, co, dt, _stream()))
    return gw


def convt_weight_forward_blocks(weight, block_offsets, blocks, ci, co):
    w = _gpu(weight, 'weight')
    dst = _gpu(blocks, 'blocks')
    if w.dtype != torch.float32 or not w.is_contiguous() or tuple(w.shape) != (ci, co, 3, 5, 5):
        raise TypeError('convt_weight_forward_blocks: weight must be a contiguous fp32 [Ci, Co, 3, 5, 5]')
    if dst.dim() != 2 or dst.stride(1) != 1 or dst.dtype not in (torch.float32, torch.bfloat16):
        raise TypeError('convt_weight_forward_blocks: blocks must be an fp32 / bf16 matrix with unit column stride')
    off = _gpu(block_offsets, 'block_offsets')
    if off.dtype != torch.int64 or tuple(off.shape) != (75, 2) or not off.is_contiguous():
        raise TypeError('convt_weight_forward_blocks: block_offsets must be a contiguous int64 [75, 2]')
    _launch('ver_convt_weight_forward_blocks', lambda: lib().ver_convt_weight_forward_blocks(
        _p(w), _p(off), dst.stride(0), _p(dst), ci, co, 1 if dst.dtype == torch.bfloat16 else 0, _stream()))
    return blocks


def _blocks_vec_args(blocks, block_rows, name):
    src = _gpu(blocks, 'blocks')
    if src.dim() != 2 or src.stride(1) != 1 or src.dtype not in (torch.float32, torch.bfloat16):
        raise TypeError('%s: blocks must be an fp32 / bf16 matrix with unit column stride' % name)
    rows = _gpu(block_rows, 'block_rows')
    if rows.dtype != torch.int64 or rows.dim() != 1 or not rows.is_contiguous():
        raise TypeError('%s: block_rows must be a contiguous int64 vector' % name)
    return src, rows


def blocks_vec_forward(blocks, block_rows, ci, x):
    src, rows = _blocks_vec_args(blocks, block_rows, 'blocks_vec_forward')
    x = _gpu(x, 'x').float().contiguous()
    if x.numel() != ci:
        raise ValueError('blocks_vec_forward: x must have Ci elements')
    part = torch.empty(8, rows.numel(), src.shape[1], dtype=torch.float32, device=src.device)
    _launch('ver_blocks_vec_forward', lambda: lib().ver_blocks_vec_forward(
        _p(src), _p(rows), rows.numel(), src.stride(0), ci, src.shape[1], _p(x), _p(part),
        1 if src.dtype == torch.bfloat16 else 0, _stream()))
    return part.sum(0)


def blocks_vec_backward(blocks, block_rows, ci, grad_vec):
    src, rows = _blocks_vec_args(blocks, block_rows, 'blocks_vec_backward')
    gv = _gpu(grad_vec, 'grad_vec').float().contiguous()
    if tuple(gv.shape) != (rows.numel(), src.shape[1]):
        raise ValueError('blocks_vec_backward: grad_vec must be [nblocks, ncols]')
    part = torch.empty(rows.numel(), ci, dtype=torch.float32, device=src.device)
    _launch('ver_blocks_vec_backward', lambda: lib().ver_blocks_vec_backward(
        _p(src), _p(rows), rows.numel(), src.stride(0), ci, src.shape[1], _p(gv), _p(part),
        1 if src.dtype == torch.bfloat16 else 0, _stream()))
    return part.sum(0)


PLAIN, PLANAR, ZSPLIT, PLANAR_ZSPLIT = 0, 1, 2, 3


def _lattice_dims(t, layout):
    s = t.shape
    if layout == PLAIN:
        return s[0], s[1], s[4]
    if layout == PLANAR:
        return s[1], s[2], s[5]
    if layout == ZSPLIT:
        return s[0], 4, s[5]
    return s[1], 4, s[6]


def lattice_transpose(channels_last, channel_first, combined_hw, layout, to_channel_first):
    cl, cf = _gpu(channels_last, 'channels_last'), _gpu(channel_first, 'channel_first')
    if not (cl.is_contiguous() and cf.is_contiguous() and cl.dtype == cf.dtype):
        raise ValueError('lattice_transpose: contiguous buffers of one dtype required')
    if cl.dtype not in (torch.float32, torch.bfloat16):
        raise TypeError('lattice_transpose: fp32 or bf16')
    H, W = combined_hw
    B, Z, C = _lattice_dims(cl, int(layout))
    dt = 1 if cl.dtype == torch.bfloat16 else 0
    _launch('ver_lattice_transpose', lambda: lib().ver_lattice_transpose(
        _p(cl), _p(cf), cf.shape[1], B, Z, H, W, C, layout, to_channel_first, dt, _stream()))


def lattice_rows(channels_last, rows, row_map, combined_hw, layout, to_rows):
    cl, buf = _gpu(channels_last, 'channels_last'), _gpu(rows, 'rows')
    if not (cl.is_contiguous() and buf.is_contiguous() and cl.dtype == torch.bfloat16 and buf.dtype == torch.bfloat16):
        raise TypeError('lattice_rows: contiguous bf16 buffers required')
    H, W = combined_hw
    B, Z, C = _lattice_dims(cl, int(layout))
    n = len(row_map['seg_off'])
    need = max(b + B * r * p for b, r, p in zip(row_map['seg_base'], row_map['seg_rows'], row_map['seg_pitch']))
    if buf.numel() < need:
        raise ValueError('lattice_rows: rows buffer of %d elements, %d needed' % (buf.numel(), need))
    ints = lambda k: (ctypes.c_int * n)(*[int(v) for v in row_map[k]])
    base = (ctypes.c_long * n)(*[int(v) for v in row_map['seg_base']])
    _launch('ver_lattice_rows', lambda: lib().ver_lattice_rows(
        _p(cl), _p(buf), row_map['quarter'], row_map['period'], n, ints('seg_off'), ints('seg_len'),
        base, ints('seg_pitch'), ints('seg_rows'), B, Z, H, W, C, layout, to_rows, 1, _stream()))


def run_gather(image, run_start, aug_idx, rows, n_rows, run_len):
    img, out = _gpu(image, 'image'), _gpu(rows, 'rows')
    if not (img.is_contiguous() and out.is_contiguous() and img.dtype == out.dtype):
        raise ValueError('run_gather: contiguous buffers of one dtype required')
    if img.dtype not in (torch.float32, torch.bfloat16):
        raise TypeError('run_gather: fp32 or bf16')
    B = img.shape[0]
    runs, n_aug = run_start.shape[1], aug_idx.shape[1]
    _launch('ver_run_gather', lambda: lib().ver_run_gather(
        _p(img), img.shape[1], _p(run_start), _p(aug_idx), _p(out), B, n_rows, runs, run_len, n_aug, out.shape[1],
        1 if img.dtype == torch.bfloat16 else 0, _stream()))


def run_scatter(rows, image, run_start, n_rows, run_len):
    src, img = _gpu(rows, 'rows'), _gpu(image, 'image')
    if not (img.is_contiguous() and src.is_contiguous() and img.dtype == src.dtype):
        raise ValueError('run_scatter: contiguous buffers of one dtype required')
    if img.dtype not in (torch.float32, torch.bfloat16):
        raise TypeError('run_scatter: fp32 or bf16')
    B = img.shape[0]
    _launch('ver_run_scatter', lambda: lib().ver_run_scatter(
        _p(src), _p(img), img.shape[1], _p(run_start), B, n_rows, run_start.shape[1], run_len,
        src.shape[1], 1 if img.dtype == torch.bfloat16 else 0, _stream()))


def _tap_args(taps, col_offset):
    flat = [int(v) for t in taps for v in t]
    return (ctypes.c_int * len(flat))(*flat), (ctypes.c_long * len(col_offset))(*[int(o) for o in col_offset])


def lattice_gather(src, col, taps, col_offset, combined_hw, layout, row_z=None, const_rows=None, const_offset=None):
    src, col = _gpu(src, 'src'), _gpu(col, 'col')
    if not (src.is_contiguous() and col.is_contiguous() and src.dtype == col.dtype):
        raise ValueError('lattice_gather: contiguous src / col of one dtype required')
    H, W = combined_hw
    B, Zs, C = _lattice_dims(src, int(layout))
    Zr = Zs if row_z is None else int(row_z)
    arr, offs = _tap_args(taps, col_offset)
    dt = 1 if src.dtype == torch.bfloat16 else 0
    cptr, coffs, nblk, cw = None, None, 0, 0
    if const_rows is not None:
        const_rows = _gpu(const_rows, 'const_rows')
        if not (const_rows.is_contiguous() and const_rows.dtype == col.dtype and const_rows.shape[0] == Zr * H * W):
            raise ValueError('lattice_gather: const_rows must be a contiguous [row_z*H*W, blocks, width] table of col.dtype')
        nblk, cw = int(const_rows.shape[1]), int(const_rows.shape[2])
        cptr, coffs = _p(const_rows), (ctypes.c_long * nblk)(*[int(o) for o in const_offset])
    _launch('ver_lattice_gather', lambda: lib().ver_lattice_gather(
        _p(src), _p(col), arr, offs, col.shape[1], len(taps), B, Zr, Zs, H, W, C, layout, dt, cptr, coffs, nblk, cw, _stream()))
    return col


def lattice_scatter(grad_col, grad_src, taps, col_offset, combined_hw, layout, row_z=None):
    grad_col, grad_src = _gpu(grad_col, 'grad_col'), _gpu(grad_src, 'grad_src')
    if not (grad_src.is_contiguous() and grad_col.is_contiguous() and grad_src.dtype == grad_col.dtype):
        raise ValueError('lattice_scatter: contiguous buffers of one dtype required')
    H, W = combined_hw
    B, Zs, C = _lattice_dims(grad_src, int(layout))
    Zr = Zs if row_z is None else int(row_z)
    arr, offs = _tap_args(taps, col_offset)
    dt = 1 if grad_src.dtype == torch.bfloat16 else 0
    _launch('ver_lattice_scatter', lambda: lib().ver_lattice_scatter(
        _p(grad_col), _p(grad_src), arr, offs, grad_col.shape[1], len(taps), B, Zr, Zs, H, W, C, layout, dt, _stream()))
    return grad_src


class LayerNormReluFunction(Function):

    @staticmethod
    def forward(ctx, x, gamma, beta, eps):
        x = _gpu(x, 'x')
        if x.dtype not in (torch.float32, torch.bfloat16):
            raise TypeError('x must be fp32 or bf16')
        w = x.shape[-1]
        n = x.numel() // w
        gamma = _gpu(gamma, 'gamma').float().contiguous()
        beta = _gpu(beta, 'beta').float().contiguous()
        dt = 1 if x.dtype == torch.bfloat16 else 0
        y = torch.empty_like(x)
        mean = torch.empty(n, dtype=torch.float32, device=x.device)
        rstd = torch.empty(n, dtype=torch.float32, device=x.device)
        _launch('ver_ln_relu_forward', lambda: lib().ver_ln_relu_forward(
            _p(x), _p(gamma), _p(beta), _p(y), _p(mean), _p(rstd), n, w, eps, dt, _stream()))
        ctx.save_for_backward(x, gamma, beta, mean, rstd)
        ctx.dt = dt
        return y

    @staticmethod
    @once_differentiable
    def backward(ctx, grad_y):
        x, gamma, beta, mean, rstd = ctx.saved_tensors
        w = x.shape[-1]
        n = x.numel() // w
        gy = _gpu(grad_y, 'grad_y').to(x.dtype).contiguous()
        gx = torch.empty_like(x)
        gg = torch.empty(w, dtype=torch.float32, device=x.device)
        gb = torch.empty(w, dtype=torch.float32, device=x.device)
        _launch('ver_ln_relu_backward', lambda: lib().ver_ln_relu_backward(
            _p(x), _p(gy), _p(gamma), _p(beta), _p(mean), _p(rstd), _p(gx), _p(gg), _p(gb), n, w, ctx.dt, _stream()))
        return gx, gg, gb, None


def layer_norm_relu(x, gamma, beta, eps=1e-5):
    return LayerNormReluFunction.apply(x, gamma, beta, eps)


class LabelRangeFlag:

    _per_device = {}

    def __init__(self, device):
        self.dev = torch.zeros(1, dtype=torch.int32, device=device)
        self.host = torch.zeros(1, dtype=torch.int32).pin_memory()
        self.event = None
        self.classes = None

    @classmethod
    def of(cls, device):
        key = (device.type, device.index if device.index is not None else torch.cuda.current_device())
        f = cls._per_device.get(key)
        if f is None:
            f = cls._per_device[key] = cls(device)
        return f

    def mirror(self, classes):
        if torch.cuda.is_current_stream_capturing():
            return
        self.classes = classes
        if self.event is not None and not self.event.query():
            return
        self.host.copy_(self.dev, non_blocking=True)
        self.event = torch.cuda.Event()
        self.event.record()

    def poll(self, sync=False):
        if torch.cuda.is_current_stream_capturing():
            return
        if sync:
            self.host.copy_(self.dev)
        elif self.event is None or not self.event.query():
            return
        if int(self.host[0]) != 0:
            raise RuntimeError(self._message())

    def _message(self):
        return ('FocalLoss: a target label outside [0, %s] reached the fused focal loss on %s (the loss of that call was '
                'NaN; F.one_hot raises on it in the reference)' % (self.classes, self.dev.device))

    def reset(self):
        self.dev.zero_()
        self.host.zero_()
        self.event = None


class AssignmentFlag(LabelRangeFlag):

    _per_device = {}

    def _message(self):
        return ('HungarianAssigner3D: a cost matrix with a NaN / -inf entry or without a finite assignment reached lsa_solve '
                'on %s (its queries were all left unmatched; scipy.optimize.linear_sum_assignment raises on it in the '
                'reference)' % (self.dev.device,))


class SigmoidFocalLossSumFunction(Function):

    @staticmethod
    def forward(ctx, logits, target, gamma, alpha):
        logits = _gpu(logits, 'logits')
        if logits.dtype not in (torch.float32, torch.bfloat16):
            raise TypeError('logits must be fp32 or bf16')
        logits = logits.contiguous()
        target = _gpu(target, 'target').to(torch.int64).contiguous()
        n, c = logits.shape
        if target.shape != (n,):
            raise ValueError('target must be [N]')
        dt = 1 if logits.dtype == torch.bfloat16 else 0
        blocks = lib().ver_focal_loss_blocks(n, c)
        partial = torch.zeros(blocks, dtype=torch.float32, device=logits.device)
        flag = LabelRangeFlag.of(logits.device)
        flag.poll()
        _launch('ver_focal_loss_forward', lambda: lib().ver_focal_loss_forward(
            _p(logits), _p(target), _p(partial), n, c, gamma, alpha, dt, _p(flag.dev), _stream()))
        flag.mirror(c)
        ctx.save_for_backward(logits, target)
        ctx.cfg = (gamma, alpha, dt)
        return partial.sum()

    @staticmethod
    @once_differentiable
    def backward(ctx, grad_out):
        logits, target = ctx.saved_tensors
        gamma, alpha, dt = ctx.cfg
        n, c = logits.shape
        scale = _gpu(grad_out, 'grad_out').float().reshape(1).contiguous()
        grad = torch.empty_like(logits)
        _launch('ver_focal_loss_backward', lambda: lib().ver_focal_loss_backward(
            _p(logits), _p(target), _p(scale), _p(grad), n, c, gamma, alpha, dt, _stream()))
        return grad, None, None, None


def sigmoid_focal_loss_sum(logits, target, gamma=2.0, alpha=0.25):
    return SigmoidFocalLossSumFunction.apply(logits, target, float(gamma), float(alpha))


def occ_mlp_pack(w1, w2, w3):
    w1, w2, w3 = (_gpu(w, 'weight').detach().float().contiguous() for w in (w1, w2, w3))
    if w1.shape != (128, 128) or w2.shape != (128, 128) or w3.shape != (16, 128):
        raise ValueError('occ_mlp is built for Linear(128,128) x2 + Linear(128,16)')
    image = torch.empty(lib().ver_occ_mlp_image_bytes() // 2, dtype=torch.bfloat16, device=w1.device)
    _launch('ver_occ_mlp_pack', lambda: lib().ver_occ_mlp_pack(_p(w1), _p(w2), _p(w3), _p(image), _stream()))
    return image


def occ_mlp_vectors(b1, g1, be1, b2, g2, be2, b3):
    vec = torch.cat([_gpu(v, 'vector').detach().float().reshape(-1) for v in (b1, g1, be1, b2, g2, be2, b3)])
    if vec.numel() != lib().ver_occ_mlp_vector_floats():
        raise ValueError('occ_mlp vectors: expected 6x128 + 16 floats')
    return vec.contiguous()


_OCC_MLP_SAVE_RSTD = os.environ.get('VER_OCC_MLP_SAVE_RSTD', '1') == '1'


def occ_mlp_forward(x, image, vectors, eps=1e-5, first_linear=True, centered=False, want_rstd=False):
    x = _gpu(x, 'x')
    if x.dtype != torch.bfloat16 or x.shape[-1] != 128:
        raise TypeError('x must be bf16 [..., 128]')
    x = x.contiguous()
    n = x.numel() // 128
    logits = torch.empty(x.shape[:-1] + (16,), dtype=torch.bfloat16, device=x.device)
    rstd = torch.empty(n, 2, dtype=torch.float32, device=x.device) if want_rstd else None
    _launch('ver_occ_mlp_forward', lambda: lib().ver_occ_mlp_forward_stats(
        _p(x), _p(image), _p(vectors), _p(logits), _p(rstd), n, 128, 16, eps,
        (1 if first_linear else 0) | (2 if centered else 0), _stream()))
    return (logits, rstd) if want_rstd else logits


def _occ_mlp_wants_rstd(folded, centered, n):
    return bool(_OCC_MLP_SAVE_RSTD and folded and centered and _OCC_MLP_BWD_FUSED and occ_mlp_backward_takes_grad_scale()
                and n < (1 << 28))


def _rows_tn(a, b, chunk=8000, with_colsum=True):
    n = a.shape[0]
    s = n // chunk
    main = s * chunk
    prod = a.new_zeros((a.shape[1], b.shape[1]), dtype=torch.float32)
    colsum = a.new_zeros((a.shape[1],), dtype=torch.float32)
    if s:
        a3 = a[:main].view(s, chunk, -1)
        prod += torch.bmm(a3.transpose(1, 2), b[:main].view(s, chunk, -1)).sum(0, dtype=torch.float32)
        if with_colsum:
            ones = a.new_ones((1, 1, chunk)).expand(s, 1, chunk)
            colsum += torch.bmm(ones, a3).sum((0, 1), dtype=torch.float32)
    if main < n:
        prod += (a[main:].t() @ b[main:]).float()
        if with_colsum:
            colsum += a[main:].sum(0, dtype=torch.float32)
    return prod, colsum


def occ_mlp_backward_takes_grad_scale():
    return os.environ.get('VER_OCC_MLP_WS', '1') not in ('0',)


_FRAG_ORDER = {}


def _frag_order(device):
    key = str(device)
    if key not in _FRAG_ORDER:
        pos = torch.arange(128)
        t, g, j = pos // 32, (pos % 32) // 8, pos % 8
        feat = 32 * t + torch.where(j < 4, 4 * g + j, 16 + 4 * g + j - 4)
        inv = torch.empty(128, dtype=torch.long)
        inv[feat] = pos
        _FRAG_ORDER[key] = inv.to(device)
    return _FRAG_ORDER[key]


_OCC_MLP_BWD_FUSED = os.environ.get('VER_OCC_MLP_BWD_FUSED', '1') == '1'


class OccMLPFunction(Function):

    @staticmethod
    def forward(ctx, x, w1, b1, g1, be1, w2, b2, g2, be2, w3, b3, eps, centered=False):
        x = _gpu(x, 'x').contiguous()
        ctx.folded = w1 is None
        if ctx.folded:
            w1, b1 = w2, torch.zeros(128, device=x.device)
        image = occ_mlp_pack(w1, w2, w3)
        vec = occ_mlp_vectors(b1, g1, be1, b2, g2, be2, b3)
        ctx.eps, ctx.centered = eps, bool(centered)
        ctx.has_rstd = _occ_mlp_wants_rstd(ctx.folded, centered, x.numel() // 128) and any(ctx.needs_input_grad)
        out = occ_mlp_forward(x, image, vec, eps, first_linear=not ctx.folded, centered=centered, want_rstd=ctx.has_rstd)
        logits, rstd = out if ctx.has_rstd else (out, None)
        ctx.save_for_backward(x, image, vec, w2.detach(), w3.detach(), *((rstd,) if ctx.has_rstd else ()))
        return logits

    @staticmethod
    @once_differentiable
    def backward(ctx, grad_logits):
        x, image, vec, w2, w3 = ctx.saved_tensors[:5]
        rstd = ctx.saved_tensors[5] if ctx.has_rstd else None
        shape = x.shape
        x2 = x.view(-1, 128)
        n = x2.shape[0]
        gl = _gpu(grad_logits, 'grad_logits').to(torch.bfloat16).contiguous().view(n, 16)
        gscale = None
        if ctx.folded and _OCC_MLP_BWD_FUSED:
            gx = torch.empty_like(x2)
            pg = torch.empty(6 * 128 + 16 * 128 + 16 + 128 * 128, dtype=torch.float32, device=x.device)
            _launch('ver_occ_mlp_backward_fused', lambda: lib().ver_occ_mlp_backward_fused_stats(
                _p(x2), _p(gl), _p(w2.float().contiguous()), _p(w3.float().contiguous()), _p(vec),
                _p(rstd), _p(gx), _p(pg), n, 128, 16, ctx.eps, _p(gscale), 2 if ctx.centered else 0, _stream()))
            vecs = pg[:768].view(6, 128)
            dw3 = pg[768:768 + 2048].view(16, 128)
            db3 = pg[768 + 2048:768 + 2048 + 16]
            dw2 = pg[768 + 2048 + 16:].view(128, 128)
            return (gx.view(shape), None, None, vecs[0], vecs[1], dw2, vecs[5], vecs[3], vecs[4], dw3, db3, None, None)
        gx, ga2, h1 = (torch.empty_like(x2) for _ in range(3))
        ga1 = None if ctx.folded else torch.empty_like(x2)
        pg = torch.empty(6 * 128 + 16 * 128 + 16, dtype=torch.float32, device=x.device)
        _launch('ver_occ_mlp_backward', lambda: lib().ver_occ_mlp_backward(
            _p(x2), _p(gl), _p(image), _p(vec), _p(gx), _p(ga1), _p(ga2), _p(h1), _p(pg),
            n, 128, 16, ctx.eps, 0 if ctx.folded else 1, _stream()))
        inv = _frag_order(x.device)
        vecs = pg[:768].view(6, 128)
        dw3 = pg[768:768 + 2048].view(16, 128)
        db3 = pg[768 + 2048:]
        dw2, _ = _rows_tn(ga2, h1, with_colsum=False)
        if ctx.folded:
            dw2 = dw2.index_select(0, inv)
            return (gx.view(shape), None, None, vecs[0], vecs[1], dw2, vecs[5], vecs[3], vecs[4], dw3, db3, None, None)
        dw2 = dw2.index_select(0, inv).index_select(1, inv)
        dw1, _ = _rows_tn(ga1, x2, with_colsum=False)
        dw1 = dw1.index_select(0, inv)
        return (gx.view(shape), dw1, vecs[2], vecs[0], vecs[1], dw2, vecs[5], vecs[3], vecs[4], dw3, db3, None, None)


class OccMLPFocalLossFunction(Function):

    @staticmethod
    def forward(ctx, x, g1, be1, w2, b2, g2, be2, w3, b3, target, eps, gamma, alpha, centered):
        x = _gpu(x, 'x').contiguous()
        image = occ_mlp_pack(w2, w2, w3)
        vec = occ_mlp_vectors(torch.zeros(128, device=x.device), g1, be1, b2, g2, be2, b3)
        ctx.has_rstd = _occ_mlp_wants_rstd(True, centered, x.numel() // 128)
        out = occ_mlp_forward(x, image, vec, eps, first_linear=False, centered=centered, want_rstd=ctx.has_rstd)
        logits, rstd = out if ctx.has_rstd else (out, None)
        l2 = logits.view(-1, 16)
        n = l2.shape[0]
        target = _gpu(target, 'target')
        as_bytes = target.dtype == torch.uint8
        target = (target if as_bytes else target.to(torch.int64)).contiguous()
        if target.shape != (n,):
            raise ValueError('target must be [N]')
        blocks = lib().ver_focal_loss_blocks(n, 16)
        partial = torch.zeros(blocks, dtype=torch.float32, device=x.device)
        flag = LabelRangeFlag.of(x.device)
        flag.poll()
        entry = lib().ver_focal_loss_forward_grad_u8 if as_bytes else lib().ver_focal_loss_forward_grad
        _launch('ver_focal_loss_forward_grad', lambda: entry(
            _p(l2), _p(target), _p(partial), _p(l2), n, 16, gamma, alpha, 1, _p(flag.dev), _stream()))
        flag.mirror(16)
        ctx.save_for_backward(x, vec, w2.detach(), w3.detach(), l2, *((rstd,) if ctx.has_rstd else ()))
        ctx.eps, ctx.centered = eps, bool(centered)
        return partial.sum()

    @staticmethod
    @once_differentiable
    def backward(ctx, grad_out):
        x, vec, w2, w3, gl = ctx.saved_tensors[:5]
        rstd = ctx.saved_tensors[5] if ctx.has_rstd else None
        shape = x.shape
        x2 = x.view(-1, 128)
        n = x2.shape[0]
        gscale = _gpu(grad_out, 'grad_out').float().reshape(1).contiguous()
        gx = torch.empty_like(x2)
        pg = torch.empty(6 * 128 + 16 * 128 + 16 + 128 * 128, dtype=torch.float32, device=x.device)
        _launch('ver_occ_mlp_backward_fused', lambda: lib().ver_occ_mlp_backward_fused_stats(
            _p(x2), _p(gl), _p(w2.float().contiguous()), _p(w3.float().contiguous()), _p(vec),
            _p(rstd), _p(gx), _p(pg), n, 128, 16, ctx.eps, _p(gscale), 2 if ctx.centered else 0, _stream()))
        vecs = pg[:768].view(6, 128)
        dw3 = pg[768:768 + 2048].view(16, 128)
        db3 = pg[768 + 2048:768 + 2048 + 16]
        dw2 = pg[768 + 2048 + 16:].view(128, 128)
        return (gx.view(shape), vecs[0], vecs[1], dw2, vecs[5], vecs[3], vecs[4], dw3, db3, None, None, None, None, None)


def occ_mlp_focal_loss_sum(x, g1, be1, w2, b2, g2, be2, w3, b3, target, eps=1e-5, gamma=2.0, alpha=0.25, centered=False):
    return OccMLPFocalLossFunction.apply(x, g1, be1, w2, b2, g2, be2, w3, b3, target, eps, float(gamma), float(alpha), centered)


def occ_mlp(x, w1, b1, g1, be1, w2, b2, g2, be2, w3, b3, eps=1e-5, centered=False):
    return OccMLPFunction.apply(x, w1, b1, g1, be1, w2, b2, g2, be2, w3, b3, eps, centered)


class AddDropoutLayerNormFunction(Function):

    @staticmethod
    def forward(ctx, a, residual, gamma, beta, p_drop, eps, want_bf16):
        a = _gpu(a, 'a')
        if a.dtype not in (torch.float32, torch.bfloat16):
            a = a.float()
        a = a.contiguous()
        res = _gpu(residual, 'residual').float().contiguous()
        C = a.shape[-1]
        n = a.numel() // C
        y = torch.empty_like(res)
        y16 = torch.empty(res.shape, dtype=torch.bfloat16, device=res.device) if want_bf16 else None
        mean = torch.empty(n, dtype=torch.float32, device=res.device)
        rstd = torch.empty_like(mean)
        seed = torch.randint(0, 2 ** 62, (1,), device=res.device, dtype=torch.int64) if p_drop > 0 else None
        g, b = gamma.detach().float().contiguous(), beta.detach().float().contiguous()
        _launch('ver_add_ln_forward', lambda: lib().ver_add_ln_forward(
            _p(a), 1 if a.dtype == torch.bfloat16 else 0, _p(res), _p(g), _p(b), _p(seed), p_drop, eps, _p(y), _p(y16),
            _p(mean), _p(rstd), n, C, _stream()))
        ctx.save_for_backward(a, res, g, mean, rstd, seed if seed is not None else torch.empty(0, device=res.device))
        ctx.p_drop, ctx.has_y16 = p_drop, want_bf16
        if want_bf16:
            return y, y16
        return y, None

    @staticmethod
    @once_differentiable
    def backward(ctx, grad_y, grad_y16):
        a, res, g, mean, rstd, seed = ctx.saved_tensors
        C = a.shape[-1]
        n = a.numel() // C
        gy = (torch.zeros_like(res) if grad_y is None else _gpu(grad_y, 'grad_y').float().contiguous())
        gy16 = None
        if ctx.has_y16 and grad_y16 is not None:
            gy16 = _gpu(grad_y16, 'grad_y_bf16').to(torch.bfloat16).contiguous()
        d_a = torch.empty_like(a)
        d_res = torch.empty_like(res)
        dg = torch.empty(C, dtype=torch.float32, device=res.device)
        db = torch.empty_like(dg)
        _launch('ver_add_ln_backward', lambda: lib().ver_add_ln_backward(
            _p(gy), _p(gy16), _p(a), 1 if a.dtype == torch.bfloat16 else 0, _p(res), _p(g), _p(mean), _p(rstd),
            _p(seed) if ctx.p_drop > 0 else None, ctx.p_drop, _p(d_a), _p(d_res), _p(dg), _p(db), n, C, _stream()))
        return d_a, d_res, dg, db, None, None, None


class ReluDropoutFunction(Function):

    @staticmethod
    def forward(ctx, x, p_drop):
        x = _gpu(x, 'x')
        if x.dtype not in (torch.float32, torch.bfloat16):
            x = x.float()
        x = x.contiguous()
        y = torch.empty_like(x)
        seed = torch.randint(0, 2 ** 62, (1,), device=x.device, dtype=torch.int64) if p_drop > 0 else None
        _launch('ver_relu_dropout_forward', lambda: lib().ver_relu_dropout_forward(
            _p(x), _p(y), _p(seed), p_drop, x.numel(), 1 if x.dtype == torch.bfloat16 else 0, _stream()))
        ctx.save_for_backward(y)
        ctx.p_drop = p_drop
        return y

    @staticmethod
    @once_differentiable
    def backward(ctx, grad_y):
        y, = ctx.saved_tensors
        gy = _gpu(grad_y, 'grad_y').to(y.dtype).contiguous()
        gx = torch.empty_like(y)
        _launch('ver_relu_dropout_backward', lambda: lib().ver_relu_dropout_backward(
            _p(y), _p(gy), _p(gx), ctx.p_drop, y.numel(), 1 if y.dtype == torch.bfloat16 else 0, _stream()))
        return gx, None


def relu_dropout(x, p_drop=0.0):
    return ReluDropoutFunction.apply(x, float(p_drop))


def add_dropout_layer_norm(a, residual, gamma, beta, p_drop=0.0, eps=1e-5, want_bf16=False):
    return AddDropoutLayerNormFunction.apply(a, residual, gamma, beta, float(p_drop), float(eps), bool(want_bf16))


class VoxelMSDeformAttnFunction(Function):

    @staticmethod
    def forward(ctx, value, spatial_shapes, level_start_index, sampling_locations, attention_weights):
        value = _gpu(value, 'value').float().contiguous()
        loc = _gpu(sampling_locations, 'sampling_locations').float().contiguous()
        aw = _gpu(attention_weights, 'attention_weights').float().contiguous()
        shapes = _gpu(spatial_shapes, 'spatial_shapes').to(torch.int64).contiguous()
        lsi = _gpu(level_start_index, 'level_start_index').to(torch.int64).contiguous()
        bs, nk, heads, hd = value.shape
        _, nq, _, nl, npt, _ = loc.shape
        out = value.new_empty(bs, nq, heads * hd)
        _launch('ver_msda3d_forward', lambda: lib().ver_msda3d_forward(
            _p(value), _p(shapes), _p(lsi), _p(loc), _p(aw), _p(out), bs, nk, heads, hd, nl, npt, nq, _stream()))
        ctx.save_for_backward(value, shapes, lsi, loc, aw)
        return out

    @staticmethod
    @once_differentiable
    def backward(ctx, grad_output):
        value, shapes, lsi, loc, aw = ctx.saved_tensors
        bs, nk, heads, hd = value.shape
        _, nq, _, nl, npt, _ = loc.shape
        gv, gl, ga = torch.zeros_like(value), torch.zeros_like(loc), torch.zeros_like(aw)
        go = _gpu(grad_output, 'grad_output').float().contiguous()
        _launch('ver_msda3d_backward', lambda: lib().ver_msda3d_backward(
            _p(value), _p(shapes), _p(lsi), _p(loc), _p(aw), _p(go), _p(gv), _p(gl), _p(ga), bs, nk, heads,
            hd, nl, npt, nq, _stream()))
        return gv, None, None, gl, ga


def voxel_msda(value, spatial_shapes, level_start_index, sampling_locations, attention_weights):
    return VoxelMSDeformAttnFunction.apply(value, spatial_shapes, level_start_index, sampling_locations,
                                           attention_weights)


def occ_predict(logits, threshold=0.25):
    logits = _gpu(logits, 'logits')
    if logits.dtype not in (torch.float32, torch.bfloat16):
        logits = logits.float()
    logits = logits.contiguous()
    n, c = logits.shape
    dt = 1 if logits.dtype == torch.bfloat16 else 0
    nb = lib().ver_occ_predict_blocks(n)
    work = torch.empty(max(nb, 1), dtype=torch.int32, device=logits.device)
    pairs = torch.empty(max(n, 1), 2, dtype=torch.int64, device=logits.device)
    count = torch.empty(1, dtype=torch.int64, device=logits.device)
    _launch('ver_occ_predict', lambda: lib().ver_occ_predict(
        _p(logits), dt, n, c, threshold, _p(work), _p(pairs), _p(count), _stream()))
    return pairs[:int(count.item())]


def occ_confusion(logits, labels, thresholds=(0.25,), samples=1, hist=None):
    logits = _gpu(logits, 'logits')
    if logits.dtype not in (torch.float32, torch.bfloat16):
        logits = logits.float()
    c = logits.shape[-1]
    logits = logits.reshape(-1, c).contiguous()
    labels = _gpu(labels, 'labels', torch.uint8).reshape(-1)
    n = logits.shape[0]
    if labels.numel() != n:
        raise ValueError('occ_confusion: %d labels for %d logit rows' % (labels.numel(), n))
    if samples < 1 or n % samples:
        raise ValueError('occ_confusion: %d rows do not split into %d samples' % (n, samples))
    thr = [float(t) for t in thresholds]
    k = c + 1
    shape = (samples, len(thr), k, k)
    if hist is None:
        hist = torch.zeros(shape, dtype=torch.int64, device=logits.device)
    elif (tuple(hist.shape) != shape or hist.dtype != torch.int64 or not hist.is_contiguous()
          or hist.device != logits.device):
        raise ValueError('occ_confusion: hist must be a contiguous int64 %s tensor on %s' % (shape, logits.device))
    dt = 1 if logits.dtype == torch.bfloat16 else 0
    host_thr = (ctypes.c_float * max(len(thr), 1))(*thr)
    _launch('ver_occ_confusion', lambda: lib().ver_occ_confusion(
        _p(logits), dt, n // samples, samples, c, _p(labels), host_thr, len(thr), _p(hist), _stream()))
    return hist


LSA_MAX = 1024


def lsa_solve(cost, ncols, match=None, bad=None):
    cost = _gpu(cost, 'cost', torch.float32)
    if cost.dim() < 2:
        raise ValueError('lsa_solve: cost must be [..., R, Ccap]')
    r, ccap = cost.shape[-2:]
    lead = tuple(cost.shape[:-2])
    n = 1
    for d in lead:
        n *= d
    ncols = _gpu(ncols, 'ncols', torch.int32).reshape(-1)
    if ncols.numel() != n:
        raise ValueError('lsa_solve: %d column counts for %d problems' % (ncols.numel(), n))
    if match is None:
        match = torch.empty(lead + (r,), dtype=torch.int32, device=cost.device)
    elif (tuple(match.shape) != lead + (r,) or match.dtype != torch.int32 or not match.is_contiguous()
          or match.device != cost.device):
        raise ValueError('lsa_solve: match must be a contiguous int32 %s tensor on %s' % (lead + (r,), cost.device))
    if bad is not None and (bad.numel() != 1 or bad.dtype != torch.int32 or bad.device != cost.device):
        raise ValueError('lsa_solve: bad must be one int32 on %s' % (cost.device,))
    if r == 0:
        return match
    _launch('ver_lsa_solve', lambda: lib().ver_lsa_solve(_p(cost), _p(ncols), _p(match), _p(bad), n, r, ccap, _stream()))
    return match


def wgrad_tn_supported(a, g):
    return (a.is_cuda and g.is_cuda and a.dtype == torch.bfloat16 and g.dtype == torch.bfloat16 and a.dim() == 2
            and g.dim() == 2 and a.shape[0] == g.shape[0] and a.stride(1) == 1 and g.stride(1) == 1
            and a.stride(0) % 8 == 0 and g.stride(0) % 8 == 0 and a.data_ptr() % 16 == 0 and g.data_ptr() % 16 == 0
            and g.shape[1] % 4 == 0)


def wgrad_tn(a, g, out_dtype=None, splits=0, flags=0, out=None):
    if not wgrad_tn_supported(a, g):
        raise RuntimeError('wgrad_tn: unsupported operands %s %s / %s %s' % (tuple(a.shape), a.stride(), tuple(g.shape), g.stride()))
    m, ka = a.shape
    n = g.shape[1]
    out_dtype = out_dtype or a.dtype
    if out_dtype not in (torch.bfloat16, torch.float32):
        raise TypeError('wgrad_tn: out_dtype must be bf16 or fp32')
    L = lib()
    if splits <= 0:
        splits = L.ver_wgrad_tn_splits_ld(m, ka, n, max(a.stride(0), g.stride(0)))
    nbytes = L.ver_wgrad_tn_workspace(m, ka, n, splits)
    ws = torch.empty(nbytes // 4, dtype=torch.float32, device=a.device)
    if out is None:
        out = torch.empty(ka, n, dtype=out_dtype, device=a.device)
    elif not (out.is_cuda and out.shape == (ka, n) and out.dtype == out_dtype and out.stride(1) == 1):
        raise RuntimeError('wgrad_tn: out must be a [Ka, N] GPU matrix of out_dtype with unit column stride')
    _launch('ver_wgrad_tn', lambda: L.ver_wgrad_tn(
        _p(a), a.stride(0), _p(g), g.stride(0), m, ka, n, _p(out), out.stride(0), 1 if out_dtype == torch.bfloat16 else 0,
        splits, flags, _p(ws), nbytes, _stream()), meta=dict(flops=2.0 * m * ka * n))
    return out


def gemm_nn_supported(a, w):
    return (a.is_cuda and w.is_cuda and a.dtype == torch.bfloat16 and w.dtype == torch.bfloat16 and a.dim() == 2
            and w.dim() == 2 and a.shape[1] == w.shape[0] and a.stride(1) == 1 and w.stride(1) == 1
            and a.stride(0) % 8 == 0 and w.stride(0) % 8 == 0 and a.data_ptr() % 16 == 0 and w.data_ptr() % 16 == 0
            and a.shape[1] % 32 == 0 and a.shape[1] >= 64)


def gemm_nn_splits(m, k, n):
    return lib().ver_gemm_nn_splits(m, k, n)


def gemm_nn(a, w, bias=None, out=None, splits=None, timer_class='ver_gemm_nn'):
    if not gemm_nn_supported(a, w):
        raise RuntimeError('gemm_nn: unsupported operands %s %s / %s %s' % (tuple(a.shape), a.stride(), tuple(w.shape), w.stride()))
    m, k = a.shape
    n = w.shape[1]
    if out is None:
        out = torch.empty(m, n, dtype=torch.bfloat16, device=a.device)
    if out.shape != (m, n) or out.dtype != torch.bfloat16 or out.stride(1) != 1 or not out.is_cuda:
        raise RuntimeError('gemm_nn: out must be a bf16 [M, N] GPU matrix with unit column stride')
    if bias is not None:
        bias = _gpu(bias, 'bias').float().contiguous()
    if splits is None:
        splits = gemm_nn_splits(m, k, n)
    if splits > 1 and (n % 4 or out.stride(0) % 4 or out.data_ptr() % 8):
        splits = 1
    ws = torch.empty(splits * m * n, dtype=torch.float32, device=a.device) if splits > 1 else None
    _launch(timer_class, lambda: lib().ver_gemm_nn_splitk(
        _p(a), a.stride(0), _p(w), w.stride(0), _p(bias), _p(out), out.stride(0), m, k, n, splits, _p(ws),
        ws.numel() * 4 if ws is not None else 0, _stream()), meta=dict(flops=2.0 * m * k * n))
    return out


def gemm_nn_taps_supported(lattice, layout, w, c):
    return (lattice.is_cuda and lattice.dtype == torch.bfloat16 and lattice.is_contiguous() and layout in (PLAIN, ZSPLIT, PLANAR_ZSPLIT)
            and lattice.numel() * 2 < 2 ** 31 - 1 and c % 32 == 0 and c >= 64
            and (w is None or (w.is_cuda and w.dtype == torch.bfloat16 and w.dim() == 2 and w.stride(1) == 1 and w.stride(0) % 8 == 0
                               and w.data_ptr() % 16 == 0)))


def gemm_nn_taps(lattice, layout, combined_hw, taps, w, rowpos=None, bias=None, out=None, const_rows=None, planes=None,
                 timer_class='ver_gemm_nn'):
    lat, w = _gpu(lattice, 'lattice'), _gpu(w, 'w')
    H, W = combined_hw
    plane_elems = nplanes = 0
    if planes is not None:
        nplanes, plane_elems = int(lat.shape[0]), int(lat[0].numel())
        if len(planes) != len(taps) or not lat.is_contiguous():
            raise ValueError('gemm_nn_taps: one source plane per tap, contiguous planes')
        B, _, C = _lattice_dims(lat[0], int(layout))
        lat_one = lat[0]
    else:
        B, _, C = _lattice_dims(lat, int(layout))
        lat_one = lat
    if not gemm_nn_taps_supported(lat_one, int(layout), w, C):
        raise RuntimeError('gemm_nn_taps: unsupported operands %s layout %d / %s %s' % (tuple(lat.shape), layout, tuple(w.shape), w.stride()))
    m, n = B * 2 * H * W, w.shape[1]
    ncst = cw = 0
    if const_rows is not None:
        const_rows = _gpu(const_rows, 'const_rows')
        if not (const_rows.is_contiguous() and const_rows.dtype == torch.bfloat16 and const_rows.dim() == 3 and const_rows.shape[0] == 2 * H * W):
            raise ValueError('gemm_nn_taps: const_rows must be a contiguous bf16 [2 H W, blocks, width] table')
        ncst, cw = int(const_rows.shape[1]), int(const_rows.shape[2])
    taps = [((-1 - int(t[1]), 0, 0) if t[0] == 'c' else t) for t in taps]
    kdim = sum(cw if t[0] < 0 else C for t in taps)
    if w.shape[0] != kdim:
        raise ValueError('gemm_nn_taps: w has %d rows, the segments span %d columns' % (w.shape[0], kdim))
    if out is None:
        out = torch.empty(m, n, dtype=torch.bfloat16, device=lat.device)
    if out.shape != (m, n) or out.dtype != torch.bfloat16 or out.stride(1) != 1 or not out.is_cuda:
        raise RuntimeError('gemm_nn_taps: out must be a bf16 [M, N] GPU matrix with unit column stride')
    if rowpos is not None:
        rowpos = _gpu(rowpos, 'rowpos').float().contiguous()
        if tuple(rowpos.shape) != (2 * H * W, n):
            raise ValueError('gemm_nn_taps: rowpos must be [2 H W, N]')
    if bias is not None:
        bias = _gpu(bias, 'bias').float().contiguous()
    flat = [int(v) for t in taps for v in t]
    arr = (ctypes.c_int * len(flat))(*flat)
    parr = (ctypes.c_int * len(taps))(*[int(v) for v in planes]) if planes is not None else None
    _launch(timer_class, lambda: lib().ver_gemm_nn_planes(
        _p(lat), layout, B, H, W, C, plane_elems, nplanes, parr, arr, len(taps), _p(const_rows), ncst, cw, _p(w), w.stride(0),
        _p(rowpos), _p(bias), _p(out), out.stride(0), n, _stream()), meta=dict(flops=2.0 * m * w.shape[0] * n))
    return out


def _segment_args(lat, layout, combined_hw, taps, const_rows, name):
    H, W = combined_hw
    B, _, C = _lattice_dims(lat, int(layout))
    ncst = cw = 0
    if const_rows is not None:
        const_rows = _gpu(const_rows, 'const_rows')
        if not (const_rows.is_contiguous() and const_rows.dtype == torch.bfloat16 and const_rows.dim() == 3 and const_rows.shape[0] == 2 * H * W):
            raise ValueError('%s: const_rows must be a contiguous bf16 [2 H W, blocks, width] table' % name)
        ncst, cw = int(const_rows.shape[1]), int(const_rows.shape[2])
    taps = [((-1 - int(t[1]), 0, 0) if t[0] == 'c' else t) for t in taps]
    kdim = sum(cw if t[0] < 0 else C for t in taps)
    flat = [int(v) for t in taps for v in t]
    return B, H, W, C, const_rows, ncst, cw, kdim, (ctypes.c_int * len(flat))(*flat), len(taps)


WGRAD_SEGMENTS_ROWS = (16, 2048)


def wgrad_tn_segments_supported(lattice, layout, combined_hw, c, const_width, g):
    H, W = combined_hw
    return (WGRAD_SEGMENTS_ROWS[0] <= 2 * H * W <= WGRAD_SEGMENTS_ROWS[1]
            and lattice.is_cuda and lattice.dtype == torch.bfloat16 and lattice.is_contiguous() and layout in (PLAIN, ZSPLIT, PLANAR_ZSPLIT)
            and lattice.numel() * 2 < 2 ** 31 - 1 and c % 64 == 0 and const_width % 64 == 0
            and (g is None or (g.is_cuda and g.dtype == torch.bfloat16 and g.dim() == 2 and g.stride(1) == 1 and g.stride(0) % 8 == 0
                               and g.data_ptr() % 16 == 0 and g.shape[1] % 4 == 0)))


def wgrad_tn_segments(lattice, layout, combined_hw, taps, g, out_dtype=None, out=None, const_rows=None, splits=0):
    lat, g = _gpu(lattice, 'lattice'), _gpu(g, 'g')
    B, H, W, C, const_rows, ncst, cw, ka, arr, nseg = _segment_args(lat, layout, combined_hw, taps, const_rows, 'wgrad_tn_segments')
    if not wgrad_tn_segments_supported(lat, int(layout), (H, W), C, cw, g):
        raise RuntimeError('wgrad_tn_segments: unsupported operands %s layout %d / %s %s' % (tuple(lat.shape), layout, tuple(g.shape), g.stride()))
    if g.shape[0] != B * 2 * H * W:
        raise ValueError('wgrad_tn_segments: g has %d rows, %d cells' % (g.shape[0], B * 2 * H * W))
    n = g.shape[1]
    out_dtype = out_dtype or (out.dtype if out is not None else lat.dtype)
    if out is None:
        out = torch.empty(ka, n, dtype=out_dtype, device=lat.device)
    elif not (out.is_cuda and out.shape == (ka, n) and out.dtype == out_dtype and out.stride(1) == 1):
        raise RuntimeError('wgrad_tn_segments: out must be a [Ka, N] GPU matrix of out_dtype with unit column stride')
    L = lib()
    if splits <= 0:
        splits = L.ver_wgrad_tn_segments_splits(B, H, W, ka, n, g.stride(0))
    ws = torch.empty(splits * ka * n, dtype=torch.float32, device=lat.device)
    _launch('ver_wgrad_tn', lambda: L.ver_wgrad_tn_segments(
        _p(lat), layout, B, H, W, C, arr, nseg, _p(const_rows), ncst, cw, _p(g), g.stride(0), n, _p(out), out.stride(0),
        1 if out_dtype == torch.bfloat16 else 0, splits, _p(ws), ws.numel() * 4, _stream()), meta=dict(flops=2.0 * g.shape[0] * ka * n))
    return out
```

Baseline: 724.6.

## Fuse split-K reduction and bias gradient into the wgrad TN kernel

The weight-gradient GEMM now reduces its split-K partials in-kernel. Each output tile has a ticket counter, and the last block to finish sums the fp32 slices and writes the output, which removes the separate reduce launch. The bias gradient (column sum of g) is also accumulated with compensated summation from the already-loaded G fragments, replacing a separate torch sum in the upsample layer-0 backward. The cost is extra epilogue work, atomics and fences, a persistent ticket buffer cached per stream, and a reduction that runs serially in the last block of each tile.

```diff
diff --git a/include/ver_ops.h b/include/ver_ops.h
--- a/include/ver_ops.h
+++ b/include/ver_ops.h
@@ -173,6 +173,16 @@
                            int ncst, int cw, const void* g, long ldg, int N, void* out, long ldo, int out_dtype, int splits,
                            void* workspace, long workspace_bytes, void* stream);
 int  ver_wgrad_tn_segments_splits(int B, int H, int W, long Ka, int N, long ldg);
+long ver_wgrad_tn_fused_workspace(long M, int Ka, int N, int splits, int with_bias);
+long ver_wgrad_tn_fused_tickets(int Ka, int N);
+int  ver_wgrad_tn_fused_zero_tickets(void* tickets, long ticket_count, void* stream);
+int  ver_wgrad_tn_fused(const void* a, long lda, const void* g, long ldg, long M, int Ka, int N, void* out, long ldo,
+                        int out_dtype, int splits, float* grad_bias, void* workspace, long workspace_bytes, void* tickets,
+                        long ticket_count, void* stream);
+int  ver_wgrad_tn_segments_fused(const void* lattice, int layout, int B, int H, int W, int C, const int* taps, int nseg,
+                                 const void* cst, int ncst, int cw, const void* g, long ldg, int N, void* out, long ldo,
+                                 int out_dtype, int splits, float* grad_bias, void* workspace, long workspace_bytes,
+                                 void* tickets, long ticket_count, void* stream);
 
 int  ver_gemm_nn(const void* a, long lda, const void* w, long ldw, const float* bias, void* c, long ldc, long M, int K,
                  int N, int flags, void* stream);
diff --git a/vln-ver_amd/csrc/ver_wgrad.hip b/vln-ver_amd/csrc/ver_wgrad.hip
--- a/vln-ver_amd/csrc/ver_wgrad.hip
+++ b/vln-ver_amd/csrc/ver_wgrad.hip
@@ -37,6 +37,9 @@
     void* out;
     long ldo;
     int out_bf16;
+    unsigned* tickets;
+    float* grad_bias;
+    float* bias_ws;
     const __bf16* lattice;
     long lattice_bytes;
     const __bf16* cst;
@@ -122,9 +125,21 @@
     ah[3] = tr_read<SB + 1536>(a1);
 }
 
-template <int PS, int KP, int PF, int IMPL>
+struct BiasLane {
+    float s[2], c[2];
+    bool on;
+};
+__device__ __forceinline__ void bias_step(BiasLane& z, int jt, const bf16x8& b) {
+    const float t = (((float)b[0] + (float)b[1]) + ((float)b[2] + (float)b[3])) + (((float)b[4] + (float)b[5]) + ((float)b[6] + (float)b[7]));
+    const float y = t - z.c[jt], n = z.s[jt] + y;
+    z.c[jt] = (n - z.s[jt]) - y;
+    z.s[jt] = n;
+}
+
+template <int PS, int KP, int PF, int IMPL, int EPI>
 __device__ __forceinline__ void phase(char* lds, f32x16 (&acc)[4][2], const WgradLane& c, __amdgpu_buffer_rsrc_t ra,
-                                      __amdgpu_buffer_rsrc_t rg, unsigned& soA, unsigned& soG, const WgradArgs& t, WTapLane& tl) {
+                                      __amdgpu_buffer_rsrc_t rg, unsigned& soA, unsigned& soG, const WgradArgs& t, WTapLane& tl,
+                                      BiasLane& bz) {
     i32x2 al[KP][4], ah[KP][4], bl[KP][2], bh[KP][2];
     int tnext = 0;
     read_slab<PS * KP>(c, al[0], ah[0], bl[0], bh[0]);
@@ -181,22 +196,102 @@
         wtap_step(t, tl, tnext);
         __builtin_amdgcn_sched_barrier(0);
     }
+    if constexpr (EPI == 2) {
+        if (bz.on) {
+#pragma unroll
+            for (int u = 0; u < KP; ++u) {
+                bias_step(bz, 0, b[u][0]);
+                bias_step(bz, 1, b[u][1]);
+            }
+        }
+        __builtin_amdgcn_sched_barrier(0);
+    }
     __builtin_amdgcn_s_barrier();
 }
 
-template <int PS, int KP, int PF, int IMPL>
+template <int PS, int KP, int PF, int IMPL, int EPI>
 __device__ __forceinline__ void phases_from(int left, char* lds, f32x16 (&acc)[4][2], const WgradLane& c,
                                             __amdgpu_buffer_rsrc_t ra, __amdgpu_buffer_rsrc_t rg, unsigned& soA, unsigned& soG,
-                                            const WgradArgs& t, WTapLane& tl) {
+                                            const WgradArgs& t, WTapLane& tl, BiasLane& bz) {
     if constexpr (PS < kRing / KP) {
         if (left > PS * KP) {
-            phase<PS, KP, PF, IMPL>(lds, acc, c, ra, rg, soA, soG, t, tl);
-            phases_from<PS + 1, KP, PF, IMPL>(left, lds, acc, c, ra, rg, soA, soG, t, tl);
-        }
-    }
-}
-
-template <int KP, int PF, int IMPL>
+            phase<PS, KP, PF, IMPL, EPI>(lds, acc, c, ra, rg, soA, soG, t, tl, bz);
+            phases_from<PS + 1, KP, PF, IMPL, EPI>(left, lds, acc, c, ra, rg, soA, soG, t, tl, bz);
+        }
+    }
+}
+
+__device__ __forceinline__ void two_sum(float& sum, float& res, float v) {
+    const float n = sum + v, vv = n - sum;
+    res += (sum - (n - vv)) + (v - vv);
+    sum = n;
+}
+
+__device__ __forceinline__ void add4(float4& a, const float4& v) {
+    a.x += v.x;
+    a.y += v.y;
+    a.z += v.z;
+    a.w += v.w;
+}
+
+__device__ __forceinline__ void reduce_tile(const WgradArgs& p, int mt, int nt, int tid) {
+    const int j = nt * kTile + 4 * (tid & 63), wrow = tid >> 6;
+    const long cs = (long)p.Ka * p.N;
+    if (j < p.N) {
+        for (int rb = 0; rb < kTile; rb += 32) {
+            const float* src[4];
+            float4 acc[4];
+            bool ok[4];
+#pragma unroll
+            for (int q = 0; q < 4; ++q) {
+                const int i = mt * kTile + rb + wrow + 8 * q;
+                ok[q] = i < p.Ka;
+                src[q] = p.ws + (long)i * p.N + j;
+                acc[q] = ok[q] ? *reinterpret_cast<const float4*>(src[q]) : make_float4(0.f, 0.f, 0.f, 0.f);
+            }
+            for (int s = 1; s < p.S; s += 4) {
+                float4 v[4][4];
+#pragma unroll
+                for (int u = 0; u < 4; ++u)
+#pragma unroll
+                    for (int q = 0; q < 4; ++q)
+                        if (s + u < p.S && ok[q]) v[u][q] = *reinterpret_cast<const float4*>(src[q] + (s + u) * cs);
+#pragma unroll
+                for (int u = 0; u < 4; ++u)
+#pragma unroll
+                    for (int q = 0; q < 4; ++q)
+                        if (s + u < p.S && ok[q]) add4(acc[q], v[u][q]);
+            }
+#pragma unroll
+            for (int q = 0; q < 4; ++q) {
+                if (!ok[q]) continue;
+                const long o = (long)(mt * kTile + rb + wrow + 8 * q) * p.ldo + j;
+                if (p.out_bf16) {
+                    typedef __bf16 bf16x4 __attribute__((ext_vector_type(4)));
+                    bf16x4 r;
+                    r.x = (__bf16)acc[q].x;
+                    r.y = (__bf16)acc[q].y;
+                    r.z = (__bf16)acc[q].z;
+                    r.w = (__bf16)acc[q].w;
+                    *reinterpret_cast<bf16x4*>(reinterpret_cast<__bf16*>(p.out) + o) = r;
+                } else {
+                    *reinterpret_cast<float4*>(reinterpret_cast<float*>(p.out) + o) = acc[q];
+                }
+            }
+        }
+    }
+    if (p.grad_bias && mt == 0 && tid < kTile && nt * kTile + tid < p.N) {
+        const int jb = nt * kTile + tid;
+        float sum = p.bias_ws[jb], res = p.bias_ws[p.N + jb];
+        for (int s = 1; s < p.S; ++s) {
+            res += p.bias_ws[(2L * s + 1) * p.N + jb];
+            two_sum(sum, res, p.bias_ws[(2L * s) * p.N + jb]);
+        }
+        p.grad_bias[jb] = sum + res;
+    }
+}
+
+template <int KP, int PF, int IMPL, int EPI>
 __device__ __forceinline__ void wgrad_body(const WgradArgs& p) {
     static_assert(PF >= KP && PF + (KP == 1 ? 2 : 4) <= kRing, "prefetch distance against the ring (WAR on the slot)");
     extern __shared__ __attribute__((aligned(1024))) char lds[];
@@ -287,6 +382,7 @@
         for (int jt = 0; jt < 2; ++jt)
 #pragma unroll
             for (int r = 0; r < 16; ++r) acc[it][jt][r] = 0.0f;
+    BiasLane bz = {{0.f, 0.f}, {0.f, 0.f}, EPI == 2 && mt == 0 && wr == 0};
 
 #pragma unroll
     for (int s = 0; s < PF; ++s) {
@@ -307,12 +403,32 @@
     if (wr == 1) __builtin_amdgcn_s_barrier();
 
     int s = 0;
-    for (; s + kRing <= nslab; s += kRing) phases_from<0, KP, PF, IMPL>(kRing, lds, acc, c, ra, rg, soA, soG, p, tl);
-    phases_from<0, KP, PF, IMPL>(nslab - s, lds, acc, c, ra, rg, soA, soG, p, tl);
+    for (; s + kRing <= nslab; s += kRing) phases_from<0, KP, PF, IMPL, EPI>(kRing, lds, acc, c, ra, rg, soA, soG, p, tl, bz);
+    phases_from<0, KP, PF, IMPL, EPI>(nslab - s, lds, acc, c, ra, rg, soA, soG, p, tl, bz);
     if (wr == 0) __builtin_amdgcn_s_barrier();
     asm volatile("s_waitcnt vmcnt(0)" ::: "memory");
 
     const int i0 = mt * kTile + 128 * wr + 4 * (lane >> 5), j0 = nt * kTile + 64 * wc + (lane & 31);
+    if constexpr (EPI == 2) {
+        if (bz.on) {
+#pragma unroll
+            for (int jt = 0; jt < 2; ++jt) {
+                const float s0 = bz.s[jt], r0 = -bz.c[jt];
+                const float s1 = __shfl_xor(s0, 32, VER_WAVE), r1 = __shfl_xor(r0, 32, VER_WAVE);
+                float sum = s0, res = r0 + r1;
+                two_sum(sum, res, s1);
+                const int j = j0 + 32 * jt;
+                if (lane < 32 && j < p.N) {
+                    if (p.S == 1) {
+                        p.grad_bias[j] = sum + res;
+                    } else {
+                        p.bias_ws[(2L * chunk) * p.N + j] = sum;
+                        p.bias_ws[(2L * chunk + 1) * p.N + j] = res;
+                    }
+                }
+            }
+        }
+    }
     if (p.S == 1 && p.out) {
 #pragma unroll
         for (int it = 0; it < 4; ++it)
@@ -344,16 +460,35 @@
                 if (i < p.Ka && j < p.N) out[(long)i * p.N + j] = acc[it][jt][r];
             }
         }
+    if constexpr (EPI > 0) {
+        int* last = reinterpret_cast<int*>(lds);
+        __builtin_amdgcn_fence(__ATOMIC_RELEASE, "agent");
+        __syncthreads();
+        if (tid == 0) {
+            const unsigned drawn = __hip_atomic_fetch_add(p.tickets + tile, 1u, __ATOMIC_RELAXED, __HIP_MEMORY_SCOPE_AGENT);
+            *last = drawn == (unsigned)(p.S - 1);
+        }
+        __syncthreads();
+        if (!*last) return;
+        __builtin_amdgcn_fence(__ATOMIC_ACQUIRE, "agent");
+        if (tid == 0) p.tickets[tile] = 0;
+        reduce_tile(p, mt, nt, tid);
+    }
 }
 
 template <int KP, int PF>
 __global__ __launch_bounds__(512) void k_wgrad_tn(WgradArgs p) {
-    wgrad_body<KP, PF, -1>(p);
+    wgrad_body<KP, PF, -1, 0>(p);
 }
 
 template <int L, int PF>
 __global__ __launch_bounds__(512) void k_wgrad_tn_seg(WgradArgs p) {
-    wgrad_body<1, PF, L>(p);
+    wgrad_body<1, PF, L, 0>(p);
+}
+
+template <int L, int EPI>
+__global__ __launch_bounds__(512) void k_wgrad_tn_fused(WgradArgs p) {
+    wgrad_body<1, 3, L, EPI>(p);
 }
 
 template <typename OT>
@@ -460,24 +595,75 @@
     return (long)splits * Ka * N * (long)sizeof(float);
 }
 
-extern "C" int ver_wgrad_tn(const void* a, long lda, const void* g, long ldg, long M, int Ka, int N, void* out, long ldo,
-                            int out_dtype, int splits, int flags, void* workspace, long workspace_bytes, void* stream) {
+namespace {
+template <int L>
+void launch_fused(const WgradArgs& p, int blocks, hipStream_t st, hipError_t& e) {
+    const int ldsb = kLdsBytes + (L >= 0 ? 4 * p.P * 4 : 0);
+    if (p.grad_bias) {
+        e = hipFuncSetAttribute((const void*)k_wgrad_tn_fused<L, 2>, hipFuncAttributeMaxDynamicSharedMemorySize, ldsb);
+        if (e == hipSuccess) hipLaunchKernelGGL((k_wgrad_tn_fused<L, 2>), dim3((unsigned)blocks), dim3(512), ldsb, st, p);
+    } else {
+        e = hipFuncSetAttribute((const void*)k_wgrad_tn_fused<L, 1>, hipFuncAttributeMaxDynamicSharedMemorySize, ldsb);
+        if (e == hipSuccess) hipLaunchKernelGGL((k_wgrad_tn_fused<L, 1>), dim3((unsigned)blocks), dim3(512), ldsb, st, p);
+    }
+}
+
+struct FusedArgs {
+    bool on;
+    float* grad_bias;
+    unsigned* tickets;
+    long ticket_count;
+};
+
+long fused_workspace_bytes(long M, int Ka, int N, int S, bool bias) {
+    if (M > 0 && S == 1) return 0;
+    if (M <= 0) return (long)Ka * N * (long)sizeof(float);
+    return ((long)S * Ka * N + (bias ? 2L * S * N : 0)) * (long)sizeof(float);
+}
+
+int fused_setup(const char* who, WgradArgs& p, const FusedArgs& f, long M, void* workspace, long workspace_bytes) {
+    VER_REQUIRE(p.S == 1 || M == 0 || (f.tickets && f.ticket_count >= p.T), VER_EINVAL, "%s: %ld ticket counters, %d needed (one per 256 x 256 output tile, zeroed)",
+                who, f.tickets ? f.ticket_count : 0L, p.T);
+    const long need = fused_workspace_bytes(M, p.Ka, p.N, p.S, f.grad_bias != nullptr);
+    VER_REQUIRE(need == 0 || (workspace && workspace_bytes >= need), VER_EINVAL, "%s: workspace of %ld bytes, %ld needed", who, workspace ? workspace_bytes : 0L, need);
+    p.tickets = f.tickets;
+    p.grad_bias = f.grad_bias;
+    p.bias_ws = p.S > 1 ? p.ws + (long)p.S * p.Ka * p.N : nullptr;
+    return VER_OK;
+}
+
+int fused_zeros(const WgradArgs& p, const FusedArgs& f, void* out, int out_dtype, void* workspace, hipStream_t st) {
+    if (int zrc = ver_zero_async(workspace, (size_t)p.Ka * p.N * sizeof(float), st)) return zrc;
+    if (f.grad_bias)
+        if (int zrc = ver_zero_async(f.grad_bias, (size_t)p.N * sizeof(float), st)) return zrc;
+    const long n4 = (long)p.Ka * p.N / 4;
+    long grid = (n4 + 255) / 256;
+    if (grid > 8192) grid = 8192;
+    if (out_dtype == VER_F32)
+        hipLaunchKernelGGL(k_wgrad_reduce<float>, dim3((unsigned)grid), dim3(256), 0, st, (const float*)workspace, (float*)out, p.ldo, 1, p.Ka, p.N);
+    else
+        hipLaunchKernelGGL(k_wgrad_reduce<__bf16>, dim3((unsigned)grid), dim3(256), 0, st, (const float*)workspace, (__bf16*)out, p.ldo, 1, p.Ka, p.N);
+    return VER_OK;
+}
+
+int wgrad_tn_impl(const char* who, const void* a, long lda, const void* g, long ldg, long M, int Ka, int N, void* out, long ldo,
+                  int out_dtype, int splits, int flags, void* workspace, long workspace_bytes, const FusedArgs& f, void* stream) {
     hipStream_t st = (hipStream_t)stream;
-    VER_REQUIRE(M >= 0 && Ka > 0 && N > 0, VER_EINVAL, "ver_wgrad_tn: bad sizes M=%ld Ka=%d N=%d", M, Ka, N);
-    VER_REQUIRE(out && workspace && ((a && g) || M == 0), VER_EINVAL, "ver_wgrad_tn: null pointer argument");
-    VER_REQUIRE(out_dtype == VER_F32 || out_dtype == VER_BF16, VER_EINVAL, "ver_wgrad_tn: out_dtype %d", out_dtype);
-    VER_REQUIRE(lda >= Ka && ldg >= N && ldo >= N, VER_EINVAL, "ver_wgrad_tn: row pitch smaller than the row");
+    VER_REQUIRE(M >= 0 && Ka > 0 && N > 0, VER_EINVAL, "%s: bad sizes M=%ld Ka=%d N=%d", who, M, Ka, N);
+    VER_REQUIRE(out && (workspace || f.on) && ((a && g) || M == 0), VER_EINVAL, "%s: null pointer argument", who);
+    VER_REQUIRE(out_dtype == VER_F32 || out_dtype == VER_BF16, VER_EINVAL, "%s: out_dtype %d", who, out_dtype);
+    VER_REQUIRE(lda >= Ka && ldg >= N && ldo >= N, VER_EINVAL, "%s: row pitch smaller than the row", who);
     VER_REQUIRE(lda % 8 == 0 && ldg % 8 == 0 && ((uintptr_t)a & 15) == 0 && ((uintptr_t)g & 15) == 0, VER_EUNSUPPORTED,
-                "ver_wgrad_tn: operands must be 16-byte aligned with row pitches that are multiples of 8 elements");
+                "%s: operands must be 16-byte aligned with row pitches that are multiples of 8 elements", who);
     VER_REQUIRE(N % 4 == 0 && ldo % 4 == 0 && ((uintptr_t)out & 15) == 0, VER_EUNSUPPORTED,
-                "ver_wgrad_tn: N and the output pitch must be multiples of 4");
+                "%s: N and the output pitch must be multiples of 4", who);
     const int S = splits > 0 ? splits : pick_splits(M, Ka, N, lda > ldg ? lda : ldg);
-    VER_REQUIRE(S <= 65536, VER_EINVAL, "ver_wgrad_tn: %d row chunks", S);
+    VER_REQUIRE(S <= 65536, VER_EINVAL, "%s: %d row chunks", who, S);
     const long Mc = ((M + S - 1) / S + 2 * kSlabRows - 1) / (2 * kSlabRows) * (2 * kSlabRows);
     VER_REQUIRE((Mc + 16 * kRing) * (lda > ldg ? lda : ldg) * 2 < 0xFFFFFFFFL, VER_EUNSUPPORTED,
-                "ver_wgrad_tn: a row chunk exceeds the 4-GiB range of a buffer offset (more splits)");
-    VER_REQUIRE(workspace_bytes >= (long)S * Ka * N * (long)sizeof(float), VER_EINVAL, "ver_wgrad_tn: workspace of %ld bytes, %ld needed",
-                workspace_bytes, (long)S * Ka * N * (long)sizeof(float));
+                "%s: a row chunk exceeds the 4-GiB range of a buffer offset (more splits)", who);
+    VER_REQUIRE(f.on || workspace_bytes >= (long)S * Ka * N * (long)sizeof(float), VER_EINVAL, "%s: workspace of %ld bytes, %ld needed",
+                who, workspace_bytes, (long)S * Ka * N * (long)sizeof(float));
     WgradArgs p = {};
     p.A = (const __bf16*)a;
     p.G = (const __bf16*)g;
@@ -492,10 +678,20 @@
     p.tiles_n = (N + kTile - 1) / kTile;
     p.T = ((Ka + kTile - 1) / kTile) * p.tiles_n;
     const bool direct = S == 1 && M > 0;
-    p.out = direct ? out : nullptr;
+    p.out = direct || f.on ? out : nullptr;
     p.ldo = ldo;
     p.out_bf16 = out_dtype == VER_BF16;
     hipError_t e = hipSuccess;
+    if (f.on) {
+        if (int rc = fused_setup(who, p, f, M, workspace, workspace_bytes)) return rc;
+        if (M > 0) {
+            launch_fused<-1>(p, p.T * S, st, e);
+            if (e != hipSuccess) return ver_fail(VER_ELAUNCH, "%s: LDS attribute: %s", who, hipGetErrorString(e));
+        } else if (int zrc = fused_zeros(p, f, out, out_dtype, workspace, st)) {
+            return zrc;
+        }
+        return ver_check_launch(who);
+    }
     if (M > 0) {
         switch (flags & 15) {
             case 4: launch_tn<1, 4>(p, p.T * S, st, e); break;
@@ -505,11 +701,11 @@
             case 8 + 4: launch_tn<2, 4>(p, p.T * S, st, e); break;
             default: launch_tn<1, 3>(p, p.T * S, st, e); break;
         }
-        if (e != hipSuccess) return ver_fail(VER_ELAUNCH, "ver_wgrad_tn: LDS attribute: %s", hipGetErrorString(e));
+        if (e != hipSuccess) return ver_fail(VER_ELAUNCH, "%s: LDS attribute: %s", who, hipGetErrorString(e));
     } else if (int zrc = ver_zero_async(workspace, (size_t)S * Ka * N * sizeof(float), st)) {
         return zrc;
     }
-    if (direct) return ver_check_launch("ver_wgrad_tn");
+    if (direct) return ver_check_launch(who);
     const long n4 = (long)Ka * N / 4;
     long grid = (n4 + 255) / 256;
     if (grid > 8192) grid = 8192;
@@ -517,55 +713,55 @@
         hipLaunchKernelGGL(k_wgrad_reduce<float>, dim3((unsigned)grid), dim3(256), 0, st, (const float*)workspace, (float*)out, ldo, S, Ka, N);
     else
         hipLaunchKernelGGL(k_wgrad_reduce<__bf16>, dim3((unsigned)grid), dim3(256), 0, st, (const float*)workspace, (__bf16*)out, ldo, S, Ka, N);
-    return ver_check_launch("ver_wgrad_tn");
-}
-
-extern "C" int ver_wgrad_tn_segments(const void* lattice, int layout, int B, int H, int W, int C, const int* taps, int nseg,
-                                     const void* cst, int ncst, int cw, const void* g, long ldg, int N, void* out, long ldo,
-                                     int out_dtype, int splits, void* workspace, long workspace_bytes, void* stream) {
+    return ver_check_launch(who);
+}
+
+int wgrad_tn_segments_impl(const char* who, const void* lattice, int layout, int B, int H, int W, int C, const int* taps, int nseg,
+                           const void* cst, int ncst, int cw, const void* g, long ldg, int N, void* out, long ldo, int out_dtype,
+                           int splits, void* workspace, long workspace_bytes, const FusedArgs& f, void* stream) {
     hipStream_t st = (hipStream_t)stream;
-    VER_REQUIRE(B >= 0 && H > 0 && W > 0 && C > 0 && N > 0 && nseg > 0, VER_EINVAL, "ver_wgrad_tn_segments: bad sizes");
-    VER_REQUIRE(layout == 0 || layout == 2 || layout == 3, VER_EINVAL, "ver_wgrad_tn_segments: layout %d (0 plain, 2 z-split, 3 planar z-split)", layout);
-    VER_REQUIRE(layout != 3 || (H % 2 == 0 && W % 2 == 0), VER_EINVAL, "ver_wgrad_tn_segments: planar needs even H, W");
-    VER_REQUIRE(out && workspace && ((lattice && g && taps) || B == 0), VER_EINVAL, "ver_wgrad_tn_segments: null pointer argument");
-    VER_REQUIRE(out_dtype == VER_F32 || out_dtype == VER_BF16, VER_EINVAL, "ver_wgrad_tn_segments: out_dtype %d", out_dtype);
-    VER_REQUIRE(nseg <= 64, VER_EUNSUPPORTED, "ver_wgrad_tn_segments: %d segments (at most 64)", nseg);
+    VER_REQUIRE(B >= 0 && H > 0 && W > 0 && C > 0 && N > 0 && nseg > 0, VER_EINVAL, "%s: bad sizes", who);
+    VER_REQUIRE(layout == 0 || layout == 2 || layout == 3, VER_EINVAL, "%s: layout %d (0 plain, 2 z-split, 3 planar z-split)", who, layout);
+    VER_REQUIRE(layout != 3 || (H % 2 == 0 && W % 2 == 0), VER_EINVAL, "%s: planar needs even H, W", who);
+    VER_REQUIRE(out && (workspace || f.on) && ((lattice && g && taps) || B == 0), VER_EINVAL, "%s: null pointer argument", who);
+    VER_REQUIRE(out_dtype == VER_F32 || out_dtype == VER_BF16, VER_EINVAL, "%s: out_dtype %d", who, out_dtype);
+    VER_REQUIRE(nseg <= 64, VER_EUNSUPPORTED, "%s: %d segments (at most 64)", who, nseg);
     VER_REQUIRE(C % 64 == 0 && (cst == nullptr || (ncst > 0 && ncst <= 64 && cw > 0 && cw % 64 == 0 && ((uintptr_t)cst & 15) == 0)),
-                VER_EUNSUPPORTED, "ver_wgrad_tn_segments: segment widths (C = %d, pattern blocks of %d) must be multiples of 64", C, cw);
+                VER_EUNSUPPORTED, "%s: segment widths (C = %d, pattern blocks of %d) must be multiples of 64", who, C, cw);
     const long M = (long)B * 2 * H * W, lbytes = (long)B * 4 * H * W * C * 2;
     const int P = 2 * H * W;
     VER_REQUIRE(P >= kSlabRows && P <= 2048 && lbytes < 0x7FFFFFFFL, VER_EUNSUPPORTED,
-                "ver_wgrad_tn_segments: %d rows per viewpoint / a source lattice of %ld bytes (16 <= rows <= 2048: four offset tables "
-                "next to the 128-KB ring in LDS; below 2 GiB)", P, lbytes);
+                "%s: %d rows per viewpoint / a source lattice of %ld bytes (16 <= rows <= 2048: four offset tables "
+                "next to the 128-KB ring in LDS; below 2 GiB)", who, P, lbytes);
     VER_REQUIRE(ldg >= N && ldo >= N && ldg % 8 == 0 && ((uintptr_t)g & 15) == 0 && ((uintptr_t)lattice & 15) == 0, VER_EUNSUPPORTED,
-                "ver_wgrad_tn_segments: g must be 16-byte aligned with a row pitch that is a multiple of 8 elements");
+                "%s: g must be 16-byte aligned with a row pitch that is a multiple of 8 elements", who);
     VER_REQUIRE(N % 4 == 0 && ldo % 4 == 0 && ((uintptr_t)out & 15) == 0, VER_EUNSUPPORTED,
-                "ver_wgrad_tn_segments: N and the output pitch must be multiples of 4");
+                "%s: N and the output pitch must be multiples of 4", who);
     WgradArgs p = {};
     long Ka = 0;
     for (int i = 0; i < nseg; ++i) {
         const int dz = taps[3 * i], dy = taps[3 * i + 1], dx = taps[3 * i + 2];
         p.seg_start[i] = (int)Ka;
         if (dz < 0) {
-            VER_REQUIRE(cst && -1 - dz < ncst, VER_EINVAL, "ver_wgrad_tn_segments: segment %d names pattern block %d of %d", i, -1 - dz, cst ? ncst : 0);
+            VER_REQUIRE(cst && -1 - dz < ncst, VER_EINVAL, "%s: segment %d names pattern block %d of %d", who, i, -1 - dz, cst ? ncst : 0);
             p.kind[i] = 1, p.dz[i] = (signed char)(-1 - dz);
             Ka += cw;
         } else {
             VER_REQUIRE((dz == 0 || dz == 2) && dy >= -64 && dy <= 64 && dx >= -64 && dx <= 64, VER_EINVAL,
-                        "ver_wgrad_tn_segments: tap %d = (%d, %d, %d): dz must be 0 or 2", i, dz, dy, dx);
+                        "%s: tap %d = (%d, %d, %d): dz must be 0 or 2", who, i, dz, dy, dx);
             p.kind[i] = 0, p.dz[i] = (signed char)dz, p.dy[i] = (signed char)dy, p.dx[i] = (signed char)dx;
             Ka += C;
         }
     }
     p.seg_start[nseg] = (int)Ka;
-    VER_REQUIRE(Ka < 0x7FFFFFFFL, VER_EUNSUPPORTED, "ver_wgrad_tn_segments: %ld columns", Ka);
+    VER_REQUIRE(Ka < 0x7FFFFFFFL, VER_EUNSUPPORTED, "%s: %ld columns", who, Ka);
     const int S = splits > 0 ? splits : pick_splits(M, (int)Ka, N, ldg);
-    VER_REQUIRE(S <= 65536, VER_EINVAL, "ver_wgrad_tn_segments: %d row chunks", S);
+    VER_REQUIRE(S <= 65536, VER_EINVAL, "%s: %d row chunks", who, S);
     const long Mc = ((M + S - 1) / S + 2 * kSlabRows - 1) / (2 * kSlabRows) * (2 * kSlabRows);
     VER_REQUIRE((Mc + 16 * kRing) * ldg * 2 < 0xFFFFFFFFL, VER_EUNSUPPORTED,
-                "ver_wgrad_tn_segments: a row chunk exceeds the 4-GiB range of a buffer offset (more splits)");
-    VER_REQUIRE(workspace_bytes >= (long)S * Ka * N * (long)sizeof(float), VER_EINVAL, "ver_wgrad_tn_segments: workspace of %ld bytes, %ld needed",
-                workspace_bytes, (long)S * Ka * N * (long)sizeof(float));
+                "%s: a row chunk exceeds the 4-GiB range of a buffer offset (more splits)", who);
+    VER_REQUIRE(f.on || workspace_bytes >= (long)S * Ka * N * (long)sizeof(float), VER_EINVAL, "%s: workspace of %ld bytes, %ld needed",
+                who, workspace_bytes, (long)S * Ka * N * (long)sizeof(float));
     p.A = nullptr;
     p.G = (const __bf16*)g;
     p.ws = (float*)workspace;
@@ -579,7 +775,7 @@
     p.tiles_n = (N + kTile - 1) / kTile;
     p.T = (int)((Ka + kTile - 1) / kTile) * p.tiles_n;
     const bool direct = S == 1 && M > 0;
-    p.out = direct ? out : nullptr;
+    p.out = direct || f.on ? out : nullptr;
     p.ldo = ldo;
     p.out_bf16 = out_dtype == VER_BF16;
     p.lattice = (const __bf16*)lattice;
@@ -588,15 +784,27 @@
     p.cst_bytes = cst ? (long)P * ncst * cw * 2 : 0;
     p.B = B, p.H = H, p.W = W, p.C = C, p.P = P, p.CW = cw, p.ncst = ncst, p.nseg = nseg;
     hipError_t e = hipSuccess;
+    if (f.on) {
+        if (int rc = fused_setup(who, p, f, M, workspace, workspace_bytes)) return rc;
+        if (M > 0) {
+            if (layout == 0) launch_fused<0>(p, p.T * S, st, e);
+            else if (layout == 2) launch_fused<2>(p, p.T * S, st, e);
+            else launch_fused<3>(p, p.T * S, st, e);
+            if (e != hipSuccess) return ver_fail(VER_ELAUNCH, "%s: LDS attribute: %s", who, hipGetErrorString(e));
+        } else if (int zrc = fused_zeros(p, f, out, out_dtype, workspace, st)) {
+            return zrc;
+        }
+        return ver_check_launch(who);
+    }
     if (M > 0) {
         if (layout == 0) launch_tn_segments<0>(p, p.T * S, st, e);
         else if (layout == 2) launch_tn_segments<2>(p, p.T * S, st, e);
         else launch_tn_segments<3>(p, p.T * S, st, e);
-        if (e != hipSuccess) return ver_fail(VER_ELAUNCH, "ver_wgrad_tn_segments: LDS attribute: %s", hipGetErrorString(e));
+        if (e != hipSuccess) return ver_fail(VER_ELAUNCH, "%s: LDS attribute: %s", who, hipGetErrorString(e));
     } else if (int zrc = ver_zero_async(workspace, (size_t)S * Ka * N * sizeof(float), st)) {
         return zrc;
     }
-    if (direct) return ver_check_launch("ver_wgrad_tn_segments");
+    if (direct) return ver_check_launch(who);
     const long n4 = Ka * N / 4;
     long grid = (n4 + 255) / 256;
     if (grid > 8192) grid = 8192;
@@ -604,7 +812,52 @@
         hipLaunchKernelGGL(k_wgrad_reduce<float>, dim3((unsigned)grid), dim3(256), 0, st, (const float*)workspace, (float*)out, ldo, S, (int)Ka, N);
     else
         hipLaunchKernelGGL(k_wgrad_reduce<__bf16>, dim3((unsigned)grid), dim3(256), 0, st, (const float*)workspace, (__bf16*)out, ldo, S, (int)Ka, N);
-    return ver_check_launch("ver_wgrad_tn_segments");
+    return ver_check_launch(who);
+}
+}
+
+extern "C" int ver_wgrad_tn(const void* a, long lda, const void* g, long ldg, long M, int Ka, int N, void* out, long ldo,
+                            int out_dtype, int splits, int flags, void* workspace, long workspace_bytes, void* stream) {
+    return wgrad_tn_impl("ver_wgrad_tn", a, lda, g, ldg, M, Ka, N, out, ldo, out_dtype, splits, flags, workspace, workspace_bytes,
+                         FusedArgs{false, nullptr, nullptr, 0}, stream);
+}
+
+extern "C" int ver_wgrad_tn_segments(const void* lattice, int layout, int B, int H, int W, int C, const int* taps, int nseg,
+                                     const void* cst, int ncst, int cw, const void* g, long ldg, int N, void* out, long ldo,
+                                     int out_dtype, int splits, void* workspace, long workspace_bytes, void* stream) {
+    return wgrad_tn_segments_impl("ver_wgrad_tn_segments", lattice, layout, B, H, W, C, taps, nseg, cst, ncst, cw, g, ldg, N, out, ldo,
+                                  out_dtype, splits, workspace, workspace_bytes, FusedArgs{false, nullptr, nullptr, 0}, stream);
+}
+
+extern "C" long ver_wgrad_tn_fused_workspace(long M, int Ka, int N, int splits, int with_bias) {
+    if (Ka <= 0 || N <= 0 || splits <= 0) return 0;
+    return fused_workspace_bytes(M, Ka, N, splits, with_bias != 0);
+}
+
+extern "C" long ver_wgrad_tn_fused_tickets(int Ka, int N) {
+    if (Ka <= 0 || N <= 0) return 0;
+    return (long)((Ka + kTile - 1) / kTile) * ((N + kTile - 1) / kTile);
+}
+
+extern "C" int ver_wgrad_tn_fused_zero_tickets(void* tickets, long ticket_count, void* stream) {
+    VER_REQUIRE(ticket_count >= 0 && (tickets || ticket_count == 0), VER_EINVAL, "ver_wgrad_tn_fused_zero_tickets: null pointer argument");
+    return ver_zero_async(tickets, (size_t)ticket_count * sizeof(unsigned), stream);
+}
+
+extern "C" int ver_wgrad_tn_fused(const void* a, long lda, const void* g, long ldg, long M, int Ka, int N, void* out, long ldo,
+                                  int out_dtype, int splits, float* grad_bias, void* workspace, long workspace_bytes,
+                                  void* tickets, long ticket_count, void* stream) {
+    return wgrad_tn_impl("ver_wgrad_tn_fused", a, lda, g, ldg, M, Ka, N, out, ldo, out_dtype, splits, 0, workspace, workspace_bytes,
+                         FusedArgs{true, grad_bias, (unsigned*)tickets, ticket_count}, stream);
+}
+
+extern "C" int ver_wgrad_tn_segments_fused(const void* lattice, int layout, int B, int H, int W, int C, const int* taps, int nseg,
+                                           const void* cst, int ncst, int cw, const void* g, long ldg, int N, void* out, long ldo,
+                                           int out_dtype, int splits, float* grad_bias, void* workspace, long workspace_bytes,
+                                           void* tickets, long ticket_count, void* stream) {
+    return wgrad_tn_segments_impl("ver_wgrad_tn_segments_fused", lattice, layout, B, H, W, C, taps, nseg, cst, ncst, cw, g, ldg, N, out,
+                                  ldo, out_dtype, splits, workspace, workspace_bytes,
+                                  FusedArgs{true, grad_bias, (unsigned*)tickets, ticket_count}, stream);
 }
 
 extern "C" int ver_wgrad_tn_segments_splits(int B, int H, int W, long Ka, int N, long ldg) {
diff --git a/vln-ver_amd/dense_heads/upsample.py b/vln-ver_amd/dense_heads/upsample.py
--- a/vln-ver_amd/dense_heads/upsample.py
+++ b/vln-ver_amd/dense_heads/upsample.py
@@ -278,14 +278,14 @@
         shape, ci, co, h, w = ctx.geom
         taps, offs, _, _ = _layer0_z4_plan(ci, operand.device)
         g = grad_out.contiguous().view(-1, 2 * co)
+        d_b = g.new_empty(2 * co, dtype=torch.float32)
         if ctx.implicit:
             from ..hipops import wgrad_tn_segments
             d_x = zs_to_plain(_dgrad_implicit('l0', g[None], wmat, shape[0], h, w, ci, co))
-            d_w = wgrad_tn_segments(operand, ZS_PLAIN, (h, w), taps, g)
+            d_w = wgrad_tn_segments(operand, ZS_PLAIN, (h, w), taps, g, grad_bias=d_b)
         else:
             d_x = _dgrad_explicit_l0(g, wmat, shape, taps, offs, ci, h, w)
-            d_w = rows_tn(operand, g)
-        d_b = g.sum(0, dtype=torch.float32)
+            d_w = rows_tn(operand, g, grad_bias=d_b)
         d_raw = convt_weight_backward_blocks(d_w, _block_offsets('l0', ci, co, d_w.device), None, None, ci, co)
         return d_x, d_raw, (d_b[:co] + d_b[co:]).to(g.dtype)
 
@@ -479,13 +479,15 @@
         return torch.addmm(b, a, w, out=out) if out is not None else torch.addmm(b, a, w)
 
 
-def rows_tn(a, g, out_dtype=None, out=None):
+def rows_tn(a, g, out_dtype=None, out=None, grad_bias=None):
     if _on_hip(a) and a.dtype == torch.bfloat16 and g.dtype == torch.bfloat16:
         from ..hipops import wgrad_tn, wgrad_tn_supported
         if g.stride(-1) != 1 or g.stride(0) % 8:
             g = g.contiguous()
         if wgrad_tn_supported(a, g):
-            return wgrad_tn(a, g, out_dtype=out_dtype if out is None else out.dtype, out=out)
+            return wgrad_tn(a, g, out_dtype=out_dtype if out is None else out.dtype, out=out, grad_bias=grad_bias)
+    if grad_bias is not None:
+        torch.sum(g, 0, dtype=grad_bias.dtype, out=grad_bias)
     if out is not None:
         return torch.mm(a.t(), g, out=out) if out.dtype == a.dtype else out.copy_(torch.mm(a.t(), g))
     res = torch.mm(a.t(), g)
diff --git a/vln-ver_amd/hipops.py b/vln-ver_amd/hipops.py
--- a/vln-ver_amd/hipops.py
+++ b/vln-ver_amd/hipops.py
@@ -1147,7 +1147,33 @@
             and g.shape[1] % 4 == 0)
 
 
-def wgrad_tn(a, g, out_dtype=None, splits=0, flags=0, out=None):
+_WGRAD_TICKETS = {}
+
+
+def _wgrad_tickets(n, device):
+    capturing = torch.cuda.is_current_stream_capturing()
+    key = (device.index, _stream())
+    buf = None if capturing else _WGRAD_TICKETS.get(key)
+    if buf is None or buf.numel() < n:
+        buf = torch.empty(max(n, 1024), dtype=torch.int32, device=device)
+        _check(lib().ver_wgrad_tn_fused_zero_tickets(_p(buf), buf.numel(), _stream()), 'ver_wgrad_tn_fused_zero_tickets')
+        if not capturing:
+            _WGRAD_TICKETS[key] = buf
+    return buf
+
+
+def _wgrad_fused_buffers(m, ka, n, splits, grad_bias, device):
+    if grad_bias is not None and not (grad_bias.is_cuda and grad_bias.dtype == torch.float32 and grad_bias.is_contiguous()
+                                      and grad_bias.numel() == n):
+        raise RuntimeError('wgrad_tn: grad_bias must be a contiguous fp32 [N] GPU vector')
+    L = lib()
+    nbytes = L.ver_wgrad_tn_fused_workspace(m, ka, n, splits, int(grad_bias is not None))
+    ws = torch.empty(nbytes // 4, dtype=torch.float32, device=device) if nbytes else None
+    tickets = _wgrad_tickets(L.ver_wgrad_tn_fused_tickets(ka, n), device) if (splits > 1 and m > 0) else None
+    return ws, nbytes, tickets, (tickets.numel() if tickets is not None else 0)
+
+
+def wgrad_tn(a, g, out_dtype=None, splits=0, flags=0, out=None, grad_bias=None):
     if not wgrad_tn_supported(a, g):
         raise RuntimeError('wgrad_tn: unsupported operands %s %s / %s %s' % (tuple(a.shape), a.stride(), tuple(g.shape), g.stride()))
     m, ka = a.shape
@@ -1158,15 +1184,23 @@
     L = lib()
     if splits <= 0:
         splits = L.ver_wgrad_tn_splits_ld(m, ka, n, max(a.stride(0), g.stride(0)))
-    nbytes = L.ver_wgrad_tn_workspace(m, ka, n, splits)
-    ws = torch.empty(nbytes // 4, dtype=torch.float32, device=a.device)
     if out is None:
         out = torch.empty(ka, n, dtype=out_dtype, device=a.device)
     elif not (out.is_cuda and out.shape == (ka, n) and out.dtype == out_dtype and out.stride(1) == 1):
         raise RuntimeError('wgrad_tn: out must be a [Ka, N] GPU matrix of out_dtype with unit column stride')
-    _launch('ver_wgrad_tn', lambda: L.ver_wgrad_tn(
+    if flags:
+        if grad_bias is not None:
+            raise RuntimeError('wgrad_tn: grad_bias needs the default pipeline shape (flags = 0)')
+        nbytes = L.ver_wgrad_tn_workspace(m, ka, n, splits)
+        ws = torch.empty(nbytes // 4, dtype=torch.float32, device=a.device)
+        _launch('ver_wgrad_tn', lambda: L.ver_wgrad_tn(
+            _p(a), a.stride(0), _p(g), g.stride(0), m, ka, n, _p(out), out.stride(0), 1 if out_dtype == torch.bfloat16 else 0,
+            splits, flags, _p(ws), nbytes, _stream()), meta=dict(flops=2.0 * m * ka * n))
+        return out
+    ws, nbytes, tickets, nt = _wgrad_fused_buffers(m, ka, n, splits, grad_bias, a.device)
+    _launch('ver_wgrad_tn', lambda: L.ver_wgrad_tn_fused(
         _p(a), a.stride(0), _p(g), g.stride(0), m, ka, n, _p(out), out.stride(0), 1 if out_dtype == torch.bfloat16 else 0,
-        splits, flags, _p(ws), nbytes, _stream()), meta=dict(flops=2.0 * m * ka * n))
+        splits, _p(grad_bias), _p(ws), nbytes, _p(tickets), nt, _stream()), meta=dict(flops=2.0 * m * ka * n))
     return out
 
 
@@ -1283,7 +1317,7 @@
                                and g.data_ptr() % 16 == 0 and g.shape[1] % 4 == 0)))
 
 
-def wgrad_tn_segments(lattice, layout, combined_hw, taps, g, out_dtype=None, out=None, const_rows=None, splits=0):
+def wgrad_tn_segments(lattice, layout, combined_hw, taps, g, out_dtype=None, out=None, const_rows=None, splits=0, grad_bias=None):
     lat, g = _gpu(lattice, 'lattice'), _gpu(g, 'g')
     B, H, W, C, const_rows, ncst, cw, ka, arr, nseg = _segment_args(lat, layout, combined_hw, taps, const_rows, 'wgrad_tn_segments')
     if not wgrad_tn_segments_supported(lat, int(layout), (H, W), C, cw, g):
@@ -1299,8 +1333,9 @@
     L = lib()
     if splits <= 0:
         splits = L.ver_wgrad_tn_segments_splits(B, H, W, ka, n, g.stride(0))
-    ws = torch.empty(splits * ka * n, dtype=torch.float32, device=lat.device)
-    _launch('ver_wgrad_tn', lambda: L.ver_wgrad_tn_segments(
+    ws, nbytes, tickets, nt = _wgrad_fused_buffers(g.shape[0], ka, n, splits, grad_bias, lat.device)
+    _launch('ver_wgrad_tn', lambda: L.ver_wgrad_tn_segments_fused(
         _p(lat), layout, B, H, W, C, arr, nseg, _p(const_rows), ncst, cw, _p(g), g.stride(0), n, _p(out), out.stride(0),
-        1 if out_dtype == torch.bfloat16 else 0, splits, _p(ws), ws.numel() * 4, _stream()), meta=dict(flops=2.0 * g.shape[0] * ka * n))
+        1 if out_dtype == torch.bfloat16 else 0, splits, _p(grad_bias), _p(ws), nbytes, _p(tickets), nt, _stream()),
+        meta=dict(flops=2.0 * g.shape[0] * ka * n))
     return out
```

After: 679.9. 6.2% lower.
